# pierrepeterlongo/commet

Hardware: AMD Instinct MI355X
Metric: reads/sec searched (index_and_search, k=32) (higher is better)
Workload: dtype u32

## Files before the change

commet_amd/csrc/capi/search_dispatch.hpp:

```cpp
#pragma once

namespace {

inline int t_eff(const commet_ctx *c, const commet_readset *rs)
{
    return (int) std::min<uint64_t>((uint64_t) c->t, (uint64_t) rs->max_len / (uint64_t) c->k + 1);
}

int launch_search(commet_ctx *c, const commet_readset *rs, const uint64_t *d_sel, uint64_t *d_tags, uint64_t *d_found,
                  unsigned long long *d_counters, unsigned long long *d_probes = nullptr, ActiveList al = ActiveList{nullptr, nullptr},
                  uint64_t n_launch = 0)
{
    if (rs->n_reads == 0) return 0;
    if (al.ids && n_launch == 0) return 0;
    const uint64_t blocks = ((al.ids ? n_launch : rs->n_reads) + 255) / 256;
    if (blocks >= (1ull << 24)) return fail("search launch too large (>= 2^32 reads in one set)");
    const dim3 g((unsigned) blocks), b(256);
    KScope ks(c, "search_kernel", c->stream);
    with_key(c->k, [&](auto key) {
        with_value<false, true>(d_probes != nullptr, [&](auto count) {
            COMMET_LAUNCH((search_kernel<decltype(key), count>), g, b, 0, c->stream, rs->view(), c->view(), c->k, t_eff(c, rs), d_sel, d_tags,
                          d_found, d_counters, d_probes, al);
        });
    });
    HIP_OK(hipGetLastError());
    return 0;
}

int ensure_slots(commet_ctx *c, int g, int gs)
{
    if (c->n_slots < g) {
        HIP_OK(hipStreamSynchronize(c->stream));
        uint32_t *nf = nullptr;
        int want = std::max(g, gs);
        hipError_t e = dev_alloc(c, (void **) &nf, (size_t) want * c->filter_bytes, true);
        if (e != hipSuccess && want > g) {
            (void) hipGetLastError();
            want = g;
            e = dev_alloc(c, (void **) &nf, (size_t) want * c->filter_bytes, true);
        }
        if (e != hipSuccess) return fail("cannot allocate %d filter slots: %s", g, hipGetErrorString(e));
        (void) dm_free(c->filter);
        c->filter = nf;
        c->n_slots = want;
    }
    if (c->il_stride < gs) {
        HIP_OK(hipStreamSynchronize(c->stream));
        (void) dm_free(c->il_a);
        c->il_a = nullptr;
        c->il_stride = 0;
        HIP_OK(dev_alloc(c, (void **) &c->il_a, (size_t) gs * c->plane_words * sizeof(uint32_t), true));
        c->il_stride = gs;
    }
    return 0;
}

int launch_interleave(commet_ctx *c, int g, int gs)
{
    const uint64_t blocks = std::min<uint64_t>((c->plane_words + 255) / 256, 1u << 16);
    KScope ks(c, "interleave_a_kernel", c->stream);
    with_value<2, 4, 8>(gs, [&](auto GS) {
        COMMET_LAUNCH(interleave_a_kernel<GS>, dim3((unsigned) blocks), dim3(256), 0, c->stream, c->filter, 4 * c->plane_words, c->plane_words,
                      g, c->il_a);
    });
    HIP_OK(hipGetLastError());
    return 0;
}

template <typename W, int GS>
int launch_search_group_t(commet_ctx *c, const commet_readset *rs, const FilterGroupView &fg, uint32_t nw_max, const uint64_t *d_sel,
                          uint64_t *d_tags, unsigned long long *d_counters, uint32_t cstride, unsigned long long *d_probes, ActiveList al,
                          uint64_t n_launch)
{
    const dim3 g((unsigned) (((al.ids ? n_launch : rs->n_reads) + 255) / 256)), b(256);
    size_t lds = (size_t) fg.g * 2 * nw_max * 256 * sizeof(uint32_t);
    uint32_t rw_nw = 0;
    if (!d_probes && nw_max <= 8 && lds + (size_t) 3 * nw_max * 256 * sizeof(uint32_t) <= (64u << 10)) {
        rw_nw = nw_max;
        lds += (size_t) 3 * nw_max * 256 * sizeof(uint32_t);
    }
    KScope ks(c, "search_group_kernel", c->stream);
    return with_value<false, true>(d_probes != nullptr, [&](auto count) {
        HIP_OK(hipFuncSetAttribute((const void *) search_group_kernel<W, GS, count>, hipFuncAttributeMaxDynamicSharedMemorySize, (int) lds));
        COMMET_LAUNCH((search_group_kernel<W, GS, count>), g, b, lds, c->stream, rs->view(), fg, c->k, t_eff(c, rs), nw_max, d_sel, d_tags,
                      d_counters, cstride, d_probes, rw_nw, al);
        HIP_OK(hipGetLastError());
        return 0;
    });
}

constexpr int MASK_MAX_WIN = 255;
inline int mask_words(const commet_ctx *c, const commet_readset *rs)
{
    const int64_t fhw = (int64_t) rs->max_len - (int64_t) t_eff(c, rs) * c->k + 1;
    return fhw <= 64 ? 2 : fhw <= 96 ? 3 : fhw <= 128 ? 4 : fhw <= 192 ? 6 : 8;
}
template <typename F>
decltype(auto) with_mask_words(int mw, F &&f)
{
    return with_value<2, 3, 4, 6, 8>(mw, f);
}

int launch_search_group(commet_ctx *c, const commet_readset *rs, int g, int gs, const uint64_t *d_sel, uint64_t *d_tags,
                        unsigned long long *d_counters, uint32_t cstride, unsigned long long *d_probes, ActiveList al = ActiveList{nullptr, nullptr},
                        uint64_t n_launch = 0, uint32_t job_mask = 0, uint64_t job_tag_words = 0)
{
    if (rs->n_reads == 0) return 0;
    if (al.ids && n_launch == 0) return 0;
    if ((rs->n_reads + 255) / 256 >= (1ull << 24)) return fail("search launch too large (>= 2^32 reads in one set)");
    FilterGroupView fg;
    fg.il_a = c->il_a;
    fg.slot0 = c->filter;
    fg.slot_words = 4 * c->plane_words;
    fg.plane_words = c->plane_words;
    fg.g = g;
    if (gs == 8) {
        const int mw_set = mask_words(c, rs);
        auto launch = [&](int mw, ActiveList l, uint64_t n_l) {
            KScope ks(c, "search_group8_kernel", c->stream);
            const dim3 grid((unsigned) (((l.ids ? n_l : rs->n_reads) + 255) / 256)), block(256);
            with_key(c->k, [&](auto key) {
                with_mask_words(mw, [&](auto MW) {
                    COMMET_LAUNCH((search_group8_kernel<decltype(key), MW>), grid, block, 0, c->stream, rs->view(), fg, c->k, t_eff(c, rs), d_sel,
                                  d_tags, d_counters, cstride, l, job_mask, job_tag_words);
                });
            });
        };
        if (al.ids && al.ids == rs->d_len_order && rs->n_len_seg > 1 && !c->mask_split) {
            for (int sg = 0; sg < rs->n_len_seg; ++sg) {
                const commet_readset::LenSeg &seg = rs->len_seg[sg];
                launch(std::min(seg.mw, mw_set), ActiveList{rs->d_len_order + seg.start, rs->d_len_order + rs->n_reads + 1 + sg}, seg.count);
            }
        } else {
            launch(mw_set, al, n_launch);
        }
        HIP_OK(hipGetLastError());
        return 0;
    }
    const uint32_t nw_max = (rs->max_len + 31) / 32;
    return with_key(c->k, [&](auto key) {
        return with_value<2, 4>(gs, [&](auto GS) {
            return launch_search_group_t<decltype(key), GS>(c, rs, fg, nw_max, d_sel, d_tags, d_counters, cstride, d_probes, al, n_launch);
        });
    });
}

bool group_searchable(const commet_ctx *c, const commet_readset *rs, int g)
{
    const uint64_t nw = ((uint64_t) rs->max_len + 31) / 32;
    return c->k >= 2 && nw >= 1 && (uint64_t) g * 2 * nw * 256 * 4 <= (64u << 10);
}

bool group8_ok(const commet_ctx *c, const commet_readset *rs)
{
    const int64_t first_hit_windows = (int64_t) rs->max_len - (int64_t) t_eff(c, rs) * c->k + 1;
    return c->k >= 2 && !c->count_probes && first_hit_windows <= MASK_MAX_WIN;
}

constexpr uint32_t LONG_MIN_MAX_LEN = 5000;
bool long_ok(const commet_ctx *c, const commet_readset *rs)
{
    if (c->long_search == 1 || c->k < 2 || rs->n_reads == 0) return false;
    if (c->long_search == 2) return true;
    const int64_t first_hit_windows = (int64_t) rs->max_len - (int64_t) t_eff(c, rs) * c->k + 1;
    if (first_hit_windows <= MASK_MAX_WIN) return false;
    return rs->max_len >= LONG_MIN_MAX_LEN;
}


int launch_search_long(commet_ctx *c, const commet_readset *rs, int g, int nf, const uint64_t *d_sel, uint64_t *d_tags,
                       unsigned long long *d_counters, uint32_t cstride, unsigned long long *d_probes, ActiveList al, uint64_t n_launch)
{
    if (rs->n_reads == 0) return 0;
    if (al.ids && n_launch == 0) return 0;
    if (g < 1 || g > nf) return fail("internal error: %d filters in a long-read pass of stride %d", g, nf);
    FilterGroupView fg;
    fg.il_a = nf == 1 ? c->slot_ptr(0) : c->il_a;
    fg.slot0 = c->filter;
    fg.slot_words = 4 * c->plane_words;
    fg.plane_words = c->plane_words;
    fg.g = g;
    const uint64_t items = al.ids ? n_launch : rs->n_reads;
    KScope ks(c, "search_long_kernel", c->stream);
    with_key(c->k, [&](auto key) {
        with_value<1, 2, 4, 8>(nf, [&](auto NF) {
            with_value<false, true>(d_probes != nullptr, [&](auto count) {
                static std::atomic<int> resident{0};
                int wgs = resident.load(std::memory_order_relaxed);
                if (!wgs) {
                    int per_cu = 0, cus = 0;
                    if (hipOccupancyMaxActiveBlocksPerMultiprocessor(&per_cu, search_long_kernel<decltype(key), NF, count>, LONG_WG, 0) != hipSuccess ||
                        hipDeviceGetAttribute(&cus, hipDeviceAttributeMultiprocessorCount, c->device) != hipSuccess || per_cu < 1 || cus < 1) {
                        (void) hipGetLastError();
                        per_cu = 4, cus = 256;
                    }
                    wgs = per_cu * cus;
                    resident.store(wgs, std::memory_order_relaxed);
                }
                const uint64_t blocks = std::min<uint64_t>((items + 3) / 4, (uint64_t) wgs);
                COMMET_LAUNCH((search_long_kernel<decltype(key), NF, count>), dim3((unsigned) blocks), dim3(LONG_WG), 0, c->stream, rs->view(), fg,
                              c->k, t_eff(c, rs), d_sel, d_tags, d_counters, cstride, d_probes, al);
            });
        });
    });
    HIP_OK(hipGetLastError());
    return 0;
}

bool sparse_pass(const commet_ctx *c, const commet_readset *rs, const uint64_t *d_sel, uint64_t selected)
{
    if (!d_sel || c->sparse_search == 1 || c->count_probes || rs->n_reads >= (1ull << 32)) return false;
    if (c->sparse_search == 2) return true;
    return rs->n_reads >= 4096 && selected * 2 < rs->n_reads;
}

int build_active_list(commet_ctx *c, const commet_readset *rs, const uint64_t *d_sel, const uint64_t *d_tags, uint64_t selected, ActiveList *al)
{
    const uint64_t n_words = bitmap_words(rs->n_reads), nb = (n_words + IDS_BLOCK_WORDS - 1) / IDS_BLOCK_WORDS;
    if (c->act_cap < selected || c->actblk_cap < nb + 1) {
        if (hipStreamSynchronize(c->stream) != hipSuccess) return 1;
        (void) dm_free(c->d_act), (void) dm_free(c->d_actblk);
        c->d_act = c->d_actblk = nullptr, c->act_cap = c->actblk_cap = 0;
        const uint64_t cap = std::max<uint64_t>(selected, 1024);
        if (dev_alloc(c, (void **) &c->d_act, cap * sizeof(uint32_t), true) != hipSuccess ||
            dev_alloc(c, (void **) &c->d_actblk, (nb + 1) * sizeof(uint32_t), true) != hipSuccess) {
            (void) hipGetLastError();
            (void) dm_free(c->d_act), (void) dm_free(c->d_actblk);
            c->d_act = c->d_actblk = nullptr;
            return 1;
        }
        c->act_cap = cap, c->actblk_cap = nb + 1;
    }
    KScope ks(c, "active_list_kernels", c->stream);
    COMMET_LAUNCH(sel_count_kernel, dim3((unsigned) nb), dim3(64), 0, c->stream, d_sel, n_words, c->d_actblk, d_tags);
    COMMET_LAUNCH(sel_scan_kernel, dim3(1), dim3(1024), 0, c->stream, c->d_actblk, (uint32_t) nb);
    COMMET_LAUNCH(sel_ids_kernel, dim3((unsigned) nb), dim3(64), 0, c->stream, d_sel, n_words, c->d_actblk, c->d_act, d_tags);
    if (hipGetLastError() != hipSuccess) return 1;
    al->ids = c->d_act;
    al->n = c->d_actblk + nb;
    return 0;
}

bool ordered_pass(commet_ctx *c, const commet_readset *rs, const uint64_t *d_sel, bool tags_empty, ActiveList *al)
{
    if (c->ordered_scan == 1 || rs->uniform_len != 0 || d_sel || !tags_empty || al->ids || c->count_probes || rs->len_order_failed) return false;
    if (rs->n_reads == 0 || rs->n_reads >= (1ull << 32) - 1 || (c->ordered_scan == 0 && rs->n_reads < (1u << 16))) return false;
    if (!rs->d_len_order) {
        const uint64_t n_blocks = (rs->n_reads + LO_BLOCK - 1) / LO_BLOCK, entries = n_blocks * LO_CLASSES;
        const uint32_t nb = (uint32_t) ((entries + 4095) / 4096);
        uint32_t *ids = nullptr;
        hipError_t e = dm_malloc((void **) &ids, (rs->n_reads + 8) * sizeof(uint32_t));
        if (e == hipSuccess && c->lo_cnt_cap < entries + 1 + nb + 2) {
            (void) dm_free(c->d_lo_cnt);
            c->d_lo_cnt = nullptr, c->lo_cnt_cap = 0;
            e = dm_malloc((void **) &c->d_lo_cnt, (entries + 1 + nb + 2) * sizeof(unsigned long long));
            if (e == hipSuccess) c->lo_cnt_cap = entries + 1 + nb + 2;
        }
        if (e != hipSuccess) {
            (void) hipGetLastError();
            (void) dm_free(ids);
            rs->len_order_failed = true;
            return false;
        }
        unsigned long long *cnt = c->d_lo_cnt, *totals = cnt + entries + 1;
        const uint32_t tk = (uint32_t) std::min<int64_t>((int64_t) t_eff(c, rs) * c->k, 0x7FFFFFFF);
        KScope ks(c, "len_order_kernels", c->stream);
        COMMET_LAUNCH(lo_count_kernel, dim3((unsigned) n_blocks), dim3(256), 0, c->stream, rs->view(), tk, n_blocks, cnt);
        COMMET_LAUNCH(tq_scan_blocks_kernel, dim3(nb), dim3(1024), 0, c->stream, cnt, entries, totals);
        COMMET_LAUNCH(tq_scan_totals_kernel, dim3(1), dim3(1024), 0, c->stream, totals, nb, totals + nb);
        COMMET_LAUNCH(tq_scan_add_kernel, dim3(nb), dim3(1024), 0, c->stream, cnt, entries, totals, totals + nb);
        COMMET_LAUNCH(lo_fill_kernel, dim3((unsigned) n_blocks), dim3(256), 0, c->stream, rs->view(), tk, n_blocks, cnt, ids);
        if (hipGetLastError() != hipSuccess) {
            (void) hipStreamSynchronize(c->stream);
            (void) dm_free(ids);
            rs->len_order_failed = true;
            return false;
        }
        rs->n_len_seg = 0;
        unsigned long long first[4] = {0, 0, 0, 0};
        static const uint32_t cls[4] = {8, 16, 20, 24};
        static const int width[5] = {8, 6, 4, 3, 2};
        bool ok = true;
        for (int i = 0; i < 4 && ok; ++i)
            ok = hipMemcpyAsync(&first[i], cnt + (uint64_t) cls[i] * n_blocks, sizeof first[i], hipMemcpyDeviceToHost, c->stream) == hipSuccess;
        ok = ok && hipStreamSynchronize(c->stream) == hipSuccess;
        if (ok) {
            const uint64_t bound[6] = {0, first[0], first[1], first[2], first[3], rs->n_reads};
            const uint64_t few = c->ordered_scan == 2 ? 1 : 4096;
            for (int i = 0; i < 5; ++i) {
                const uint64_t a = bound[i], b = bound[i + 1];
                if (b <= a || b > rs->n_reads) continue;
                if (rs->n_len_seg > 0 && b - a < few)
                    rs->len_seg[rs->n_len_seg - 1].count += (uint32_t) (b - a);
                else
                    rs->len_seg[rs->n_len_seg++] = commet_readset::LenSeg{(uint32_t) a, (uint32_t) (b - a), width[i]};
            }
            uint32_t counts[5] = {0, 0, 0, 0, 0};
            for (int i = 0; i < rs->n_len_seg; ++i) counts[i] = rs->len_seg[i].count;
            ok = hipMemcpyAsync(ids + rs->n_reads + 1, counts, sizeof counts, hipMemcpyHostToDevice, c->stream) == hipSuccess &&
                 hipStreamSynchronize(c->stream) == hipSuccess;
        }
        if (!ok) {
            (void) hipGetLastError();
            rs->n_len_seg = 0;
        }
        rs->d_len_order = ids;
    }
    al->ids = rs->d_len_order;
    al->n = rs->d_len_order + rs->n_reads;
    return true;
}

constexpr int TQ_SLICE_BITS = 24;

constexpr int TQ_MAX_K = 34;

bool tiled_ok(const commet_ctx *c, const commet_readset *rs, int g)
{
    if (c->tiled_mode == 1 || c->count_probes || rs->ql.failed) return false;
    if (c->k <= TQ_SLICE_BITS || c->k > TQ_MAX_K || g < 1 || g > 2) return false;
    const int64_t first_hit_windows = (int64_t) rs->max_len - (int64_t) t_eff(c, rs) * c->k + 1;
    if (first_hit_windows < 1 || first_hit_windows > TQ_MAX_WIN) return false;
    if (rs->max_len >= TQ_MAX_LEN) return false;
    if (rs->n_reads >= (1ull << 32)) return false;
    if (rs->fhw_total >= (1ull << 32)) return false;
    if (c->tiled_mode == 2) return true;
    const uint64_t est = rs->fhw_total * 8;
    const bool set_aside = rs->ql_reserved.load() && rs->ql_reserved_at.load() == g_devmem.trims.load();
    if (rs->n_reads < (1ull << 20) || (est > c->ql_max_list && !set_aside)) return false;
    if (est > (4ull << 30) && !rs->ql.built && rs->ql_wanted++ == 0) return false;
    return true;
}

int build_query_list(commet_ctx *c, const commet_readset *rs)
{
    commet_readset::QueryList &ql = rs->ql;
    if (ql.built) {
        ql.last_use = ++c->ql_clock;
        return 0;
    }
    ql.sbits = TQ_SLICE_BITS;
    ql.n_slices = 1u << (c->k - ql.sbits);
    ql.n_pieces = (uint32_t) ((rs->n_reads + TQ_PIECE - 1) / TQ_PIECE);
    const uint64_t entries = (uint64_t) ql.n_slices * ql.n_pieces;
    const uint32_t nb = (uint32_t) ((entries + 4095) / 4096);
    hipStream_t ls = c->list_stream;
    unsigned long long *d_totals = nullptr;
    auto alloc = [&](void **ptr, size_t bytes) -> hipError_t {
        hipError_t ae = dm_malloc(ptr, bytes);
        if (ae != hipErrorOutOfMemory) return ae;
        (void) hipGetLastError();
        if (!shrink_query_lists(c, 0, false)) return ae;
        ae = dm_malloc(ptr, bytes);
        if (ae == hipErrorOutOfMemory) (void) hipGetLastError();
        return ae;
    };
    hipError_t e = alloc((void **) &ql.d_tile_off, (entries + 1) * sizeof(unsigned long long));
    if (e == hipSuccess && c->ql_totals_cap < (uint64_t) nb + 1) {
        (void) dm_free(c->d_ql_totals);
        c->d_ql_totals = nullptr, c->ql_totals_cap = 0;
        e = alloc((void **) &c->d_ql_totals, ((size_t) nb + 1) * sizeof(unsigned long long));
        if (e == hipSuccess) c->ql_totals_cap = (uint64_t) nb + 1;
    }
    d_totals = c->d_ql_totals;
    if (e == hipSuccess) {
        const int t = t_eff(c, rs);
        const size_t lds = (size_t) ql.n_slices * 4;
        {
            KScope ks(c, "tq_count_kernel", ls);
            with_key(c->k, [&](auto key) {
                COMMET_LAUNCH(tq_count_kernel<decltype(key)>, dim3(ql.n_pieces), dim3(256), lds, ls, rs->view(), c->k, t, ql.sbits, ql.n_slices,
                              ql.n_pieces, ql.d_tile_off);
            });
        }
        {
            KScope ks(c, "tq_scan_kernels", ls);
            COMMET_LAUNCH(tq_scan_blocks_kernel, dim3(nb), dim3(1024), 0, ls, ql.d_tile_off, entries, d_totals);
            COMMET_LAUNCH(tq_scan_totals_kernel, dim3(1), dim3(1024), 0, ls, d_totals, nb, d_totals + nb);
            COMMET_LAUNCH(tq_scan_add_kernel, dim3(nb), dim3(1024), 0, ls, ql.d_tile_off, entries, d_totals, d_totals + nb);
        }
        e = hipGetLastError();
        unsigned long long total = 0;
        if (e == hipSuccess) e = hipMemcpyAsync(&total, d_totals + nb, sizeof total, hipMemcpyDeviceToHost, ls);
        if (e == hipSuccess) e = hipStreamSynchronize(ls);
        ql.n_records = total;
        if (e == hipSuccess && total >= (1ull << 32)) e = hipErrorOutOfMemory;
        if (e == hipSuccess) e = alloc((void **) &ql.d_qaddr, std::max<uint64_t>(total, 1) * 4);
        if (e == hipSuccess) e = alloc((void **) &ql.d_qwho, std::max<uint64_t>(total, 1) * 2);
        if (e == hipSuccess) e = alloc((void **) &ql.d_tstart, std::max<uint64_t>(entries, 1) * 4);
        if (e == hipSuccess) e = alloc((void **) &ql.d_tlen, std::max<uint64_t>(entries, 1) * 2);
        if (e == hipSuccess) {
            KScope ks(c, "tq_bounds_kernel", ls);
            COMMET_LAUNCH(tq_bounds_kernel, dim3((unsigned) ((entries + 255) / 256)), dim3(256), 0, ls, ql.d_tile_off, ql.n_slices,
                               ql.n_pieces, ql.d_tstart, ql.d_tlen);
            e = hipGetLastError();
        }
        if (e == hipSuccess) {
            const int64_t fhw = std::max<int64_t>(1, (int64_t) rs->max_len - (int64_t) t * c->k + 1);
            const uint32_t rounds = (uint32_t) (((uint64_t) TQ_PIECE * (uint64_t) fhw + TQ_FILL_CAP - 1) / TQ_FILL_CAP);
            uint32_t rpr = (TQ_PIECE + rounds - 1) / rounds;
            while (rpr > 1 && (uint64_t) rpr * (uint64_t) fhw > TQ_FILL_CAP) --rpr;
            const size_t lds_fill = ((size_t) 4 * ql.n_slices + 2 * TQ_FILL_CAP) * 4;
            e = with_key(c->k, [&](auto key) {
                hipError_t fe = hipFuncSetAttribute((const void *) tq_fill_kernel<decltype(key)>, hipFuncAttributeMaxDynamicSharedMemorySize, (int) lds_fill);
                if (fe != hipSuccess) return fe;
                KScope ks(c, "tq_fill_kernel", ls);
                COMMET_LAUNCH(tq_fill_kernel<decltype(key)>, dim3(ql.n_pieces), dim3(256), lds_fill, ls, rs->view(), c->k, t, ql.sbits, ql.n_slices,
                              ql.n_pieces, rpr, ql.d_tstart, ql.d_qaddr, ql.d_qwho);
                return hipGetLastError();
            });
        }
    }
    if (e == hipSuccess) e = hipEventRecord(c->ev_list, ls);
    if (e == hipSuccess) e = hipStreamWaitEvent(c->stream, c->ev_list, 0);
    if (e != hipSuccess) {
        (void) hipGetLastError();
        ql.release();
        ql.failed = true;
        return 1;
    }
    ql.built = true;
    ql.bytes = (entries + 1) * 8 + ql.n_records * 6 + entries * 6;
    ql.last_use = ++c->ql_clock;
    c->ql_bytes += ql.bytes;
    if (c->ql_bytes > c->ql_budget) (void) shrink_query_lists(c, c->ql_budget, false);
    return 0;
}

int ensure_query_results(commet_ctx *c, const commet_readset *rs)
{
    const uint64_t need = rs->ql.n_records;
    if (c->qres_cap >= need && c->d_qres) return 0;
    if (hipStreamSynchronize(c->stream) != hipSuccess) return 1;
    (void) dm_free(c->d_qres);
    c->d_qres = nullptr, c->qres_cap = 0;
    hipError_t e = dm_malloc((void **) &c->d_qres, std::max<uint64_t>(need, 1));
    if (e == hipErrorOutOfMemory) {
        (void) hipGetLastError();
        if (shrink_query_lists(c, 0, false)) e = dm_malloc((void **) &c->d_qres, std::max<uint64_t>(need, 1));
    }
    if (e != hipSuccess) {
        (void) hipGetLastError();
        rs->ql.failed = true;
        return 1;
    }
    c->qres_cap = need;
    return 0;
}

bool query_list_blocks(const commet_ctx *c, const commet_readset *rs, uint64_t out[6])
{
    const int t = t_eff(c, rs);
    const int64_t fhw = (int64_t) rs->max_len - (int64_t) t * c->k + 1;
    if (c->k <= TQ_SLICE_BITS || c->k > TQ_MAX_K || fhw < 1 || fhw > TQ_MAX_WIN || rs->max_len >= TQ_MAX_LEN || rs->n_reads < (1ull << 20) || rs->n_reads >= (1ull << 32)) return false;
    const uint64_t records = rs->fhw_total;
    if (records >= (1ull << 32)) return false;
    const uint64_t entries = ((uint64_t) 1 << (c->k - TQ_SLICE_BITS)) * ((rs->n_reads + TQ_PIECE - 1) / TQ_PIECE);
    out[0] = (entries + 1) * 8, out[1] = records * 4, out[2] = records * 2, out[3] = entries * 4, out[4] = entries * 2;
    out[5] = c->qres_cap >= records ? 0 : records;
    return true;
}

constexpr unsigned TQ_PROBE_WGS_PER_XCD = 64;

int launch_search_tiled(commet_ctx *c, const commet_readset *rs, int g, int slot0, const uint64_t *d_sel, uint64_t *d_tags,
                        unsigned long long *d_counters, uint32_t cstride, uint64_t job_tag_words = 0)
{
    if (rs->n_reads == 0) return 0;
    const commet_readset::QueryList &q = rs->ql;
    if (c->qres_cap < q.n_records) return fail("internal error: tiled search without its result buffer");
    QueryListView v;
    v.tile_off = q.d_tile_off, v.qaddr = q.d_qaddr, v.qwho = q.d_qwho, v.tstart = q.d_tstart, v.tlen = q.d_tlen;
    v.n_slices = q.n_slices, v.n_pieces = q.n_pieces, v.sbits = q.sbits;
    FilterGroupView fg;
    fg.slot0 = c->slot_ptr(slot0);
    fg.il_a = g == 1 ? c->slot_ptr(slot0) : c->il_a;
    fg.slot_words = 4 * c->plane_words;
    fg.plane_words = c->plane_words;
    fg.g = g;
    const int mw = mask_words(c, rs);
    const int t = t_eff(c, rs);
    {
        KScope ks(c, "tq_probe_kernel", c->stream);
        with_value<1, 2>(g, [&](auto GS) {
            COMMET_LAUNCH(tq_probe_kernel<GS>, dim3(8 * TQ_PROBE_WGS_PER_XCD), dim3(256), 0, c->stream, v, fg.il_a, c->d_qres, 0u, q.n_pieces);
        });
    }
    HIP_OK(hipGetLastError());
    {
        KScope ks(c, "tq_replay_kernel", c->stream);
        const uint32_t hit_cap = (uint32_t) std::min<int>(c->tq_hit_cap, TQ_HIT_CAP);
        with_key(c->k, [&](auto key) {
            with_value<1, 2>(g, [&](auto GS) {
                with_mask_words(mw, [&](auto MW) {
                    COMMET_LAUNCH((tq_replay_kernel<decltype(key), GS, MW>), dim3(q.n_pieces), dim3(TQ_PIECE), 0, c->stream, rs->view(), v, c->d_qres,
                                  fg, c->k, t, d_sel, d_tags, d_counters, cstride, 0u, hit_cap, job_tag_words);
                });
            });
        });
    }
    HIP_OK(hipGetLastError());
    return 0;
}

int slice_words(const commet_ctx *c, uint64_t n_chunks)
{
    if (c->slice_mode == 1 || c->count_probes) return 0;
    if (c->k < SLICE_MIN_K || c->k > SLICE_MAX_K || n_chunks == 0) return 0;
    if (c->slice_mode == 0 && n_chunks < 8) return 0;
    int gw = c->slice_gw ? c->slice_gw : n_chunks > 128 ? 8 : n_chunks > 64 ? 4 : n_chunks > 32 ? 2 : 1;
    while (gw > 1 && (((uint64_t) 16 * gw) << c->k) > (1ull << 30)) gw /= 2;
    return gw;
}

int ensure_slice_buffers(commet_ctx *c, int gw, uint64_t n_chunks)
{
    const uint64_t G = 32ull * gw;
    const uint64_t stage_words = (G * 4) << (c->k - 5), table_words = ((uint64_t) 4 * gw) << c->k;
    if (c->slice_stage_words < stage_words || c->slice_table_words < table_words || c->slice_chunks_cap < n_chunks) {
        HIP_OK(hipStreamSynchronize(c->stream));
        if (c->slice_stage_words < stage_words) {
            (void) dm_free(c->slice_stage);
            c->slice_stage = nullptr, c->slice_stage_words = 0;
            HIP_OK(dev_alloc(c, (void **) &c->slice_stage, stage_words * 4, true));
            c->slice_stage_words = stage_words;
        }
        if (c->slice_table_words < table_words) {
            (void) dm_free(c->slice_tables);
            c->slice_tables = nullptr, c->slice_table_words = 0;
            HIP_OK(dev_alloc(c, (void **) &c->slice_tables, table_words * 4, true));
            c->slice_table_words = table_words;
        }
        if (c->slice_chunks_cap < n_chunks) {
            (void) dm_free(c->d_slice_chunks);
            c->d_slice_chunks = nullptr, c->slice_chunks_cap = 0;
            HIP_OK(dev_alloc(c, (void **) &c->d_slice_chunks, n_chunks * sizeof(SliceChunk), true));
            c->slice_chunks_cap = n_chunks;
        }
    }
    return 0;
}

int launch_slice_build(commet_ctx *c, const commet_readset *rs, const uint64_t *d_sel, uint64_t ci, int g, int gw,
                       uint32_t *tables = nullptr, uint32_t row_words = 0, uint32_t col0 = 0)
{
    if (!tables) tables = c->slice_tables, row_words = (uint32_t) gw, col0 = 0;
    const int tile_bits = std::min(c->k, SLICE_TILE_BITS);
    const uint32_t tiles = 1u << (c->k - tile_bits);
    const size_t lds = (size_t) 4 << (tile_bits - 5);
    HIP_OK(hipFuncSetAttribute((const void *) slice_build_kernel, hipFuncAttributeMaxDynamicSharedMemorySize, (int) lds));
    {
        KScope ks(c, "slice_build_kernel", c->stream);
        COMMET_LAUNCH(slice_build_kernel, dim3(4 * tiles, (unsigned) g), dim3(1024), lds, c->stream, rs->view(), d_sel,
                           c->d_slice_chunks + ci, c->k, tile_bits, tiles, c->slice_stage);
    }
    HIP_OK(hipGetLastError());
    const unsigned grid = (unsigned) ((((uint64_t) 4 << (c->k - 5)) + 255) / 256);
    {
        KScope ks(c, "slice_transpose_kernel", c->stream);
        with_value<1, 2, 4, 8>(gw, [&](auto GW) {
            COMMET_LAUNCH(slice_transpose_kernel<GW>, dim3(grid), dim3(256), 0, c->stream, c->slice_stage, c->k, g, tables, row_words, col0);
        });
    }
    HIP_OK(hipGetLastError());
    return 0;
}

int launch_search_sliced(commet_ctx *c, const commet_readset *rs, int g, int gw, const uint64_t *d_sel, uint64_t *d_tags,
                         unsigned long long *d_counters, uint32_t cstride, uint32_t block_stride = 1)
{
    if (rs->n_reads == 0) return 0;
    if ((rs->n_reads + 255) / 256 >= (1ull << 24)) return fail("search launch too large (>= 2^32 reads in one set)");
    const uint64_t blocks = (rs->n_reads + 255) / 256;
    const dim3 grid((unsigned) ((blocks + block_stride - 1) / block_stride)), block(256);
    KScope ks(c, "search_sliced_kernel", c->stream);
    with_value<1, 2, 4, 8>(gw, [&](auto GW) {
        COMMET_LAUNCH(search_sliced_kernel<GW>, grid, block, 0, c->stream, rs->view(), c->slice_tables, c->k, t_eff(c, rs), g, d_sel, d_tags,
                      d_counters, cstride, block_stride);
    });
    HIP_OK(hipGetLastError());
    return 0;
}

struct WidePlan {
    uint32_t nw = 0;
    uint32_t rw = 0;
    uint64_t chunks_per_pass = 0;
    int lpr = 0, np = 0;
};

WidePlan wide_plan(const commet_ctx *c, uint64_t n_chunks, int slice_gw)
{
    WidePlan w;
    if (!slice_gw || c->slice_wide == 1) return w;
    if (c->slice_wide == 0 && n_chunks <= 256) return w;
    const uint64_t groups = (n_chunks + 255) / 256;
    size_t free_b = 0, total_b = 0;
    if (hipMemGetInfo(&free_b, &total_b) != hipSuccess) return w;
    const uint64_t have = (uint64_t) c->wide_table_words * 4 + dm_filed_bytes(c->device);
    const uint64_t budget = std::min<uint64_t>(((uint64_t) free_b + have) / 3, 48ull << 30);
    uint64_t cap = std::min<uint64_t>(WIDE_MAX_ROW_WORDS, budget / (16ull << c->k));
    if (c->wide_cap_words) cap = std::min<uint64_t>(cap, c->wide_cap_words);
    cap = cap / WIDE_GROUP_WORDS * WIDE_GROUP_WORDS;
    if (cap < WIDE_GROUP_WORDS) return w;
    const uint64_t passes = (groups * WIDE_GROUP_WORDS + cap - 1) / cap;
    const uint64_t groups_per_pass = (groups + passes - 1) / passes;
    w.nw = (uint32_t) (groups_per_pass * WIDE_GROUP_WORDS);
    w.rw = (w.nw + 31u) & ~31u;
    w.chunks_per_pass = groups_per_pass * 256;
    const uint32_t pieces = w.nw / 4;
    w.lpr = pieces <= 8 ? 8 : pieces <= 16 ? 16 : pieces <= 32 ? 32 : 64;
    w.np = pieces <= 64 ? 1 : 2;
    return w;
}

int ensure_wide_tables(commet_ctx *c, const WidePlan &w)
{
    const uint64_t words = ((uint64_t) 4 * w.rw) << c->k;
    if (c->wide_table_words >= words) return 0;
    HIP_OK(hipStreamSynchronize(c->stream));
    (void) dm_free(c->wide_tables);
    c->wide_tables = nullptr, c->wide_table_words = 0;
    if (dev_alloc(c, (void **) &c->wide_tables, words * 4, true) != hipSuccess) {
        (void) hipGetLastError();
        return 1;
    }
    c->wide_table_words = words;
    return 0;
}

int launch_search_wide(commet_ctx *c, const commet_readset *rs, const WidePlan &w, int g, const uint64_t *d_sel, uint64_t *d_tags,
                       unsigned long long *d_counters, uint32_t cstride)
{
    if (rs->n_reads == 0) return 0;
    const uint64_t reads_per_block = 4ull * (64 / w.lpr);
    const uint64_t blocks = (rs->n_reads + reads_per_block - 1) / reads_per_block;
    if (blocks >= (1ull << 31)) return fail("search launch too large");
    const dim3 grid((unsigned) blocks), block(256);
    const int t = t_eff(c, rs);
    KScope ks(c, "search_wide_kernel", c->stream);
    auto launch = [&](auto LPR, auto NP) {
        COMMET_LAUNCH((search_wide_kernel<LPR, NP>), grid, block, 0, c->stream, rs->view(), c->wide_tables, c->k, t, g, w.nw, w.rw, d_sel, d_tags,
                      d_counters, cstride);
    };
    if (w.np == 2) launch(std::integral_constant<int, 64>{}, std::integral_constant<int, 2>{});
    else with_value<64, 32, 16, 8>(w.lpr, [&](auto LPR) { launch(LPR, std::integral_constant<int, 1>{}); });
    HIP_OK(hipGetLastError());
    return 0;
}

}

extern "C" {

uint64_t commet_readset_cache_estimate(commet_ctx *c, const commet_readset *rs)
{
    uint64_t b[6];
    if (rs->ctx != c || !rs->finalized || !query_list_blocks(c, rs, b)) return 0;
    return b[0] + b[1] + b[2] + b[3] + b[4];
}

int commet_readset_reserve_cache(commet_ctx *c, const commet_readset *rs)
{
    if (rs->ctx != c) return fail("read set belongs to another context");
    if (!rs->finalized) return fail("read set not finalized");
    SetUse use(c, rs);
    if (use.enter()) return 1;
    HIP_OK(hipSetDevice(c->device));
    uint64_t b[6];
    {
        std::lock_guard<std::mutex> lk(c->ql_mu);
        const bool still = rs->ql_reserved.load() && rs->ql_reserved_at.load() == g_devmem.trims.load();
        if (rs->ql.built || still || !g_devmem.enabled() || !query_list_blocks(c, rs, b)) return 0;
    }
    for (int i = 0; i < 6; ++i)
        if (b[i] && dm_reserve((size_t) b[i]) != hipSuccess) return 0;
    rs->ql_reserved_at.store(g_devmem.trims.load());
    rs->ql_reserved.store(true);
    return 0;
}

}
```

commet_amd/csrc/capi/state.hpp:

```cpp
#pragma once

using namespace commet;

namespace {

thread_local std::string g_err;

std::mutex g_launch_mu;
std::set<const void *> g_launched;
inline void note_launch(const void *entry)
{
    thread_local const void *recent[16] = {nullptr};
    thread_local unsigned next = 0;
    for (const void *r : recent)
        if (r == entry) return;
    recent[next++ & 15u] = entry;
    std::lock_guard<std::mutex> lk(g_launch_mu);
    g_launched.insert(entry);
}
#define COMMET_LAUNCH(kernel, ...)                                   \
    do {                                                              \
        static std::atomic<bool> noted_{false};                       \
        if (!noted_.load(std::memory_order_relaxed)) {                \
            note_launch((const void *) (kernel));                     \
            noted_.store(true, std::memory_order_relaxed);            \
        }                                                             \
        hipLaunchKernelGGL(kernel, __VA_ARGS__);                      \
    } while (0)

template <typename F>
decltype(auto) with_key(int k, F &&f)
{
    if (k <= 32) return f(uint32_t{});
    return f(uint64_t{});
}
template <auto V, auto... Vs, typename T, typename F>
decltype(auto) with_value(T v, F &&f)
{
    if constexpr (sizeof...(Vs) == 0) {
        return f(std::integral_constant<decltype(V), V>{});
    } else {
        if (v == V) return f(std::integral_constant<decltype(V), V>{});
        return with_value<Vs...>(v, f);
    }
}

struct DevMemCache {
    struct Block {
        int device;
        size_t bytes;
        bool pooled;
    };
    std::mutex mu;
    std::map<void *, Block> live;
    std::multimap<size_t, std::pair<void *, bool>> filed[16];
    size_t filed_bytes[16] = {0};
    size_t cap[16] = {0};
    hipStream_t pool_stream[16] = {nullptr};
    int on = -1, pool_on = -1;
    size_t pool_min = 0;
    std::atomic<uint64_t> drv_ns[16], drv_bytes[16], drv_calls[16];
    std::atomic<uint64_t> trims{0};
    DevMemCache()
    {
        for (int d = 0; d < 16; ++d) drv_ns[d] = 0, drv_bytes[d] = 0, drv_calls[d] = 0;
    }
    bool enabled()
    {
        if (on < 0) {
            const char *e = getenv("COMMET_DEVMEM_CACHE");
            on = !(e && atoi(e) == 0);
        }
        return on != 0;
    }
    int verb = -1;
    bool verbose()
    {
        if (verb < 0) {
            const char *e = getenv("COMMET_DEVMEM_VERBOSE");
            verb = e && atoi(e) != 0;
        }
        return verb != 0;
    }
    bool pooling()
    {
        if (pool_on < 0) {
            const char *e = getenv("COMMET_DEVMEM_POOL");
            pool_on = e && atoi(e) != 0;
            const char *m = getenv("COMMET_DEVMEM_POOL_MIN_MB");
            pool_min = m ? std::max<size_t>((size_t) atoll(m) << 20, (size_t) 8 << 20) : (size_t) 256 << 20;
        }
        return pool_on != 0;
    }
};
DevMemCache g_devmem;
constexpr size_t DEVMEM_MIN_FILED = (size_t) 8 << 20;

hipError_t dm_driver_alloc_untimed(void **p, size_t bytes, int dev, bool shareable, bool *pooled);
hipError_t dm_driver_alloc(void **p, size_t bytes, int dev, bool shareable, bool *pooled)
{
    const auto t0 = std::chrono::steady_clock::now();
    const hipError_t e = dm_driver_alloc_untimed(p, bytes, dev, shareable, pooled);
    if (dev >= 0 && dev < 16) {
        g_devmem.drv_ns[dev] += (uint64_t) std::chrono::duration_cast<std::chrono::nanoseconds>(std::chrono::steady_clock::now() - t0).count();
        g_devmem.drv_calls[dev] += 1;
        if (e == hipSuccess) g_devmem.drv_bytes[dev] += bytes;
    }
    return e;
}
hipError_t dm_driver_alloc_untimed(void **p, size_t bytes, int dev, bool shareable, bool *pooled)
{
    *pooled = false;
    if (!shareable && g_devmem.pooling() && bytes >= g_devmem.pool_min) {
        hipStream_t st;
        {
            std::lock_guard<std::mutex> lk(g_devmem.mu);
            if (!g_devmem.pool_stream[dev] && hipStreamCreateWithFlags(&g_devmem.pool_stream[dev], hipStreamNonBlocking) != hipSuccess) {
                (void) hipGetLastError();
                g_devmem.pool_stream[dev] = nullptr;
            }
            st = g_devmem.pool_stream[dev];
        }
        if (st) {
            hipError_t e = hipMallocAsync(p, bytes, st);
            if (e == hipSuccess) e = hipStreamSynchronize(st);
            if (e == hipSuccess) {
                *pooled = true;
                return e;
            }
            if (e != hipErrorOutOfMemory) (void) hipGetLastError();
            else return e;
        }
    }
    return hipMalloc(p, bytes);
}

void dm_driver_free(void *q, int dev, bool pooled)
{
    if (!pooled) {
        (void) hipFree(q);
        return;
    }
    hipStream_t st = g_devmem.pool_stream[dev];
    (void) hipFreeAsync(q, st);
    (void) hipStreamSynchronize(st);
}

size_t dm_trim(int device)
{
    g_devmem.trims += 1;
    std::vector<std::pair<int, std::pair<void *, bool>>> drop;
    size_t bytes = 0;
    {
        std::lock_guard<std::mutex> lk(g_devmem.mu);
        for (int d = 0; d < 16; ++d) {
            if (device >= 0 && d != device) continue;
            for (auto &b : g_devmem.filed[d]) drop.push_back({d, b.second}), bytes += b.first;
            g_devmem.filed[d].clear();
            g_devmem.filed_bytes[d] = 0;
        }
    }
    bool any_pooled = false;
    for (auto &q : drop) dm_driver_free(q.second.first, q.first, q.second.second), any_pooled |= q.second.second;
    if (any_pooled) {
        int cur = 0;
        const bool have = hipGetDevice(&cur) == hipSuccess;
        for (int d = 0; d < 16; ++d) {
            if ((device >= 0 && d != device) || !g_devmem.pool_stream[d]) continue;
            hipMemPool_t pool;
            if (hipSetDevice(d) == hipSuccess && hipDeviceGetDefaultMemPool(&pool, d) == hipSuccess) (void) hipMemPoolTrimTo(pool, 0);
        }
        if (have) (void) hipSetDevice(cur);
        (void) hipGetLastError();
    }
    return bytes;
}

size_t dm_filed_bytes(int device)
{
    std::lock_guard<std::mutex> lk(g_devmem.mu);
    return device >= 0 && device < 16 ? g_devmem.filed_bytes[device] : 0;
}

size_t dm_pooled_bytes(int device)
{
    std::lock_guard<std::mutex> lk(g_devmem.mu);
    size_t n = 0;
    for (auto &b : g_devmem.live)
        if (b.second.device == device && b.second.pooled) n += b.second.bytes;
    return n;
}

inline size_t dm_size_class(size_t bytes)
{
    if (bytes < DEVMEM_MIN_FILED) return bytes;
    const int lg = 63 - __builtin_clzll((unsigned long long) bytes);
    const size_t granule = (size_t) 1 << (lg - 4);
    return (bytes + granule - 1) & ~(granule - 1);
}

hipError_t dm_malloc(void **p, size_t bytes, bool shareable = false)
{
    *p = nullptr;
    if (g_devmem.enabled()) bytes = dm_size_class(bytes);
    int dev = 0;
    if (hipGetDevice(&dev) != hipSuccess || dev < 0 || dev >= 16) return hipMalloc(p, bytes);
    if (!g_devmem.enabled()) {
        const auto t0 = std::chrono::steady_clock::now();
        const hipError_t e = hipMalloc(p, bytes);
        g_devmem.drv_ns[dev] += (uint64_t) std::chrono::duration_cast<std::chrono::nanoseconds>(std::chrono::steady_clock::now() - t0).count();
        g_devmem.drv_calls[dev] += 1;
        if (e == hipSuccess) g_devmem.drv_bytes[dev] += bytes;
        return e;
    }
    if (bytes >= DEVMEM_MIN_FILED) {
        std::lock_guard<std::mutex> lk(g_devmem.mu);
        for (auto it = g_devmem.filed[dev].lower_bound(bytes); it != g_devmem.filed[dev].end() && it->first <= bytes + bytes / 4; ++it) {
            if (shareable && it->second.second) continue;
            *p = it->second.first;
            g_devmem.filed_bytes[dev] -= it->first;
            g_devmem.live[*p] = {dev, it->first, it->second.second};
            g_devmem.filed[dev].erase(it);
            return hipSuccess;
        }
    }
    bool pooled = false;
    if (g_devmem.verbose()) {
        std::lock_guard<std::mutex> lk(g_devmem.mu);
        fprintf(stderr, "[devmem] driver alloc %.1f MiB (filed: %.1f GiB in %zu blocks)\n", bytes / 1048576.0, g_devmem.filed_bytes[dev] / 1073741824.0, g_devmem.filed[dev].size());
    }
    hipError_t e = dm_driver_alloc(p, bytes, dev, shareable, &pooled);
    if (e == hipErrorOutOfMemory && dm_trim(dev)) {
        (void) hipGetLastError();
        e = dm_driver_alloc(p, bytes, dev, shareable, &pooled);
    }
    if (e == hipSuccess && bytes >= DEVMEM_MIN_FILED) {
        std::lock_guard<std::mutex> lk(g_devmem.mu);
        g_devmem.live[*p] = {dev, bytes, pooled};
    }
    return e;
}

hipError_t dm_reserve(size_t bytes)
{
    if (!g_devmem.enabled() || bytes < DEVMEM_MIN_FILED) return hipSuccess;
    bytes = dm_size_class(bytes);
    int dev = 0;
    if (hipGetDevice(&dev) != hipSuccess || dev < 0 || dev >= 16) return hipErrorInvalidDevice;
    void *p = nullptr;
    bool pooled = false;
    const hipError_t e = dm_driver_alloc(&p, bytes, dev, false, &pooled);
    if (e != hipSuccess) {
        (void) hipGetLastError();
        return e;
    }
    std::lock_guard<std::mutex> lk(g_devmem.mu);
    g_devmem.filed[dev].emplace(bytes, std::make_pair(p, pooled));
    g_devmem.filed_bytes[dev] += bytes;
    return hipSuccess;
}

hipError_t dm_free(void *p)
{
    if (!p) return hipSuccess;
    if (g_devmem.enabled()) {
        DevMemCache::Block what{-1, 0, false};
        {
            std::lock_guard<std::mutex> lk(g_devmem.mu);
            auto it = g_devmem.live.find(p);
            if (it != g_devmem.live.end()) what = it->second, g_devmem.live.erase(it);
        }
        if (what.device >= 0) {
            const int d = what.device;
            int cur = d;
            const bool have_cur = hipGetDevice(&cur) == hipSuccess;
            if (have_cur && cur != d) (void) hipSetDevice(d);
            (void) hipDeviceSynchronize();
            std::vector<std::pair<void *, bool>> over;
            {
                std::lock_guard<std::mutex> lk(g_devmem.mu);
                g_devmem.filed[d].emplace(what.bytes, std::make_pair(p, what.pooled));
                g_devmem.filed_bytes[d] += what.bytes;
                if (!g_devmem.cap[d]) {
                    size_t fr = 0, tot = 0;
                    const char *e = getenv("COMMET_DEVMEM_CACHE_GB");
                    if (e) g_devmem.cap[d] = (size_t) (std::max(0.0, atof(e)) * (double) (1ull << 30)) + 1;
                    else g_devmem.cap[d] = hipMemGetInfo(&fr, &tot) == hipSuccess ? tot / 2 : (size_t) 64 << 30;
                }
                while (g_devmem.filed_bytes[d] > g_devmem.cap[d] && !g_devmem.filed[d].empty()) {
                    auto last = std::prev(g_devmem.filed[d].end());
                    over.push_back(last->second);
                    g_devmem.filed_bytes[d] -= last->first;
                    g_devmem.filed[d].erase(last);
                }
            }
            if (!over.empty() && g_devmem.verbose()) fprintf(stderr, "[devmem] over the cap of %.1f GiB: %zu block(s) back to the driver\n", g_devmem.cap[d] / 1073741824.0, over.size());
            for (auto &q : over) dm_driver_free(q.first, d, q.second);
            if (have_cur && cur != d) (void) hipSetDevice(cur);
            return hipSuccess;
        }
    }
    return hipFree(p);
}

hipError_t dm_make_shareable(void **p)
{
    if (!*p) return hipSuccess;
    DevMemCache::Block what{-1, 0, false};
    {
        std::lock_guard<std::mutex> lk(g_devmem.mu);
        auto it = g_devmem.live.find(*p);
        if (it != g_devmem.live.end()) what = it->second;
    }
    if (what.device < 0 || !what.pooled) return hipSuccess;
    void *q = nullptr;
    hipError_t e = dm_malloc(&q, what.bytes, true);
    if (e != hipSuccess) return e;
    e = hipDeviceSynchronize();
    if (e == hipSuccess) e = hipMemcpy(q, *p, what.bytes, hipMemcpyDeviceToDevice);
    if (e == hipSuccess) e = hipDeviceSynchronize();
    if (e != hipSuccess) {
        (void) dm_free(q);
        return e;
    }
    (void) dm_free(*p);
    *p = q;
    return hipSuccess;
}

int fail(const char *fmt, ...)
{
    char buf[1024];
    va_list ap;
    va_start(ap, fmt);
    vsnprintf(buf, sizeof buf, fmt, ap);
    va_end(ap);
    g_err = buf;
    return 1;
}

#define HIP_OK(expr)                                                                                   \
    do {                                                                                               \
        hipError_t e_ = (expr);                                                                        \
        if (e_ != hipSuccess) return fail("%s failed: %s (%s:%d)", #expr, hipGetErrorString(e_), __FILE__, __LINE__); \
    } while (0)

#define HIP_OK_NULL(expr)                                                                              \
    do {                                                                                               \
        hipError_t e_ = (expr);                                                                        \
        if (e_ != hipSuccess) {                                                                        \
            fail("%s failed: %s (%s:%d)", #expr, hipGetErrorString(e_), __FILE__, __LINE__);           \
            return nullptr;                                                                            \
        }                                                                                              \
    } while (0)

inline uint64_t bitmap_words(uint64_t n) { return n / 64 + 1; }
inline uint64_t bitmap_bytes_host(uint64_t n) { return n / 8 + 1; }

constexpr uint64_t STAGE_BASES = 64ull << 20;
constexpr uint64_t STAGE_READS = 1ull << 20;
constexpr int      N_COUNTERS = 8;

}

struct commet_ctx {
    int device = 0;
    int k = 0, t = 0;
    hipStream_t stream = nullptr;
    uint32_t *filter = nullptr;
    uint64_t plane_words = 0;
    uint64_t filter_bytes = 0;
    unsigned long long *d_counters = nullptr;
    unsigned long long *h_counters = nullptr;
    hipEvent_t ev_i0 = nullptr, ev_i1 = nullptr, ev_s0 = nullptr, ev_s1 = nullptr;
    bool have_index_ev = false, have_search_ev = false;
    bool count_probes = false;
    int index_mode = 0;
    int part_packed = 1;
    int part_no_uni = 0;
    int part_list = 0;
    uint64_t part_min_kmers = 8ull << 20;
    struct PartWs {
        uint32_t *bufA = nullptr, *bufB = nullptr;
        uint64_t cap_keys = 0, cap_b = 0;
        uint32_t *hist = nullptr, *wl = nullptr;
        uint64_t *off = nullptr, *goff = nullptr;
        unsigned long long *cur2 = nullptr, *blockoff = nullptr;
        uint32_t *blockcnt = nullptr;
        uint32_t *items = nullptr, *itemblk = nullptr;
        uint64_t items_cap = 0, itemblk_cap = 0;
        uint64_t items_set = 0, items_first = 0, items_count = 0;
        uint32_t items_nblk = 0;
        uint32_t nb = 0;
        void release()
        {
            (void) dm_free(bufA); (void) dm_free(bufB); (void) dm_free(hist); (void) dm_free(wl); (void) dm_free(off); (void) dm_free(goff);
            (void) dm_free(cur2); (void) dm_free(blockoff); (void) dm_free(blockcnt); (void) dm_free(items); (void) dm_free(itemblk);
            *this = PartWs();
        }
    } part[2];
    unsigned long long *d_jobcnt = nullptr;
    uint32_t *d_ids = nullptr, *d_idblk = nullptr;
    uint64_t ids_cap = 0, idblk_cap = 0;
    uint32_t *d_ids2 = nullptr, *d_idblk2 = nullptr;
    uint64_t ids2_cap = 0, idblk2_cap = 0;
    uint32_t *d_act = nullptr, *d_actblk = nullptr;
    uint64_t act_cap = 0, actblk_cap = 0;
    uint64_t *d_mtags = nullptr;
    uint64_t mtags_cap = 0;
    int multi_job = 0;
    int sparse_search = 0;
    unsigned long long *d_plansum = nullptr;
    uint64_t plansum_cap = 0;
    uint64_t jobcnt_cap = 0;
    hipStream_t aux_stream = nullptr;
    hipStream_t load_stream = nullptr;
    hipEvent_t ev_fork = nullptr, ev_join = nullptr;
    int index_lanes = 2;
    bool stagger_armed = false;
    hipEvent_t ev_stagger = nullptr;

    int n_slots = 1;
    int cur_slot = 0;
    uint32_t *il_a = nullptr;
    int il_stride = 0;
    struct KernelClock {
        struct Rec { const char *name; hipEvent_t a, b; };
        bool on = false;
        std::vector<Rec> open;
        std::vector<hipEvent_t> spare;
        std::vector<std::string> names;
        std::vector<uint64_t> launches;
        std::vector<double> total_ms;
        std::mutex mu;
        void add(const char *name, double ms)
        {
            std::lock_guard<std::mutex> lk(mu);
            size_t i = 0;
            while (i < names.size() && names[i] != name) ++i;
            if (i == names.size()) names.push_back(name), launches.push_back(0), total_ms.push_back(0);
            launches[i] += 1;
            total_ms[i] += ms;
        }
        hipEvent_t get()
        {
            hipEvent_t e = nullptr;
            if (!spare.empty()) e = spare.back(), spare.pop_back();
            else if (hipEventCreate(&e) != hipSuccess) e = nullptr;
            return e;
        }
        void collect()
        {
            for (Rec &r : open) {
                float ms = 0;
                if (r.a && r.b && hipEventElapsedTime(&ms, r.a, r.b) == hipSuccess) add(r.name, ms);
                if (r.a) spare.push_back(r.a);
                if (r.b) spare.push_back(r.b);
            }
            open.clear();
        }
        void reset()
        {
            std::lock_guard<std::mutex> lk(mu);
            names.clear(), launches.clear(), total_ms.clear();
        }
        void release()
        {
            collect();
            for (hipEvent_t e : spare) (void) hipEventDestroy(e);
            spare.clear();
        }
    } kclock;
    uint32_t *slice_stage = nullptr, *slice_tables = nullptr;
    SliceChunk *d_slice_chunks = nullptr;
    uint64_t slice_stage_words = 0, slice_table_words = 0, slice_chunks_cap = 0;
    hipStream_t list_stream = nullptr;
    hipEvent_t ev_list = nullptr;
    unsigned long long *d_ql_totals = nullptr;
    uint64_t ql_totals_cap = 0;
    uint8_t *d_qres = nullptr;
    uint64_t qres_cap = 0;
    int tq_hit_cap = TQ_HIT_CAP;
    int ordered_scan = 0;
    int mask_split = 0;
    unsigned long long *d_lo_cnt = nullptr;
    uint64_t lo_cnt_cap = 0;
    int tiled_mode = 0;
    bool job_verbose = false;
    bool ingest_verbose = false;
    int slice_mode = 0;
    int slice_gw = 0;
    int slice_wide = 0;
    uint32_t wide_cap_words = 0;
    uint32_t *wide_tables = nullptr;
    uint64_t wide_table_words = 0;
    uint64_t max_kmer_test = 0;
    double *d_shannon = nullptr;
    uint32_t shannon_lo = 0, shannon_hi = 0;
    int long_search = 0;
    int chunk_group = 8;
    struct IngestBuf {
        uint32_t *h_planes = nullptr;
        uint64_t *h_goff = nullptr;
        hipEvent_t done = nullptr;
    };
    std::vector<IngestBuf> ingest_pool;
    struct AwayStage {
        uint8_t *h = nullptr;
        hipEvent_t done = nullptr;
        bool inflight = false;
    } away[2];

    std::mutex ql_mu;
    std::vector<commet_readset *> sets;
    uint64_t ql_bytes = 0, ql_budget = 64ull << 30, ql_clock = 0, ql_evictions = 0;
    uint64_t ql_max_list = 4ull << 30;

    uint32_t *slot_ptr(int i) const { return filter + (uint64_t) i * 4 * plane_words; }
    FilterView view() const
    {
        uint32_t *base = slot_ptr(cur_slot);
        FilterView f;
        f.a = base;
        f.b = base + plane_words;
        f.c = base + 2 * plane_words;
        f.d = base + 3 * plane_words;
        return f;
    }
};

struct commet_readset {
    commet_ctx *ctx = nullptr;
    uint64_t max_reads = 0, max_bases = 0;
    uint64_t n_reads = 0, n_bases = 0;
    uint32_t *d_planes = nullptr;
    uint64_t *d_goff = nullptr;
    uint32_t *d_kcnt = nullptr;
    uint32_t *d_lenmm = nullptr;
    uint64_t *d_sel = nullptr, *d_tags = nullptr, *d_found = nullptr;
    struct Stage {
        uint8_t *h_bases = nullptr;
        uint64_t *h_offs = nullptr;
        uint8_t *d_bases = nullptr;
        uint64_t *d_offs = nullptr;
        hipEvent_t done = nullptr;
        bool inflight = false;
    } st[2];
    int cur = 0;
    bool acquired = false;
    uint64_t stage_bases = 0, stage_reads = 0;
    std::vector<FileSpan> files;
    std::vector<uint64_t> empty_reads;
    mutable std::vector<uint32_t> h_kcnt;
    mutable std::vector<uint64_t> h_kprefix;
    mutable bool have_host_counts = false;
    uint32_t uniform_len = 0;
    uint32_t max_kcnt = 0;
    uint32_t max_len = 0, min_len = 0;
    uint64_t uid = 0;
    uint64_t fhw_total = 0;
    struct QueryList {
        unsigned long long *d_tile_off = nullptr;
        uint32_t *d_qaddr = nullptr, *d_tstart = nullptr;
        uint16_t *d_qwho = nullptr, *d_tlen = nullptr;
        uint64_t n_records = 0;
        uint32_t n_slices = 0, n_pieces = 0;
        int sbits = 0;
        bool built = false, failed = false;
        uint64_t bytes = 0, last_use = 0;
        void release()
        {
            (void) dm_free(d_tile_off); (void) dm_free(d_qaddr); (void) dm_free(d_qwho); (void) dm_free(d_tstart); (void) dm_free(d_tlen);
            *this = QueryList();
        }
    };
    mutable QueryList ql;
    mutable uint32_t *d_len_order = nullptr;
    mutable bool len_order_failed = false;
    struct LenSeg { uint32_t start, count; int mw; };
    mutable LenSeg len_seg[5];
    mutable int n_len_seg = 0;
    mutable uint32_t ql_wanted = 0;
    mutable std::atomic<uint64_t> ql_reserved_at{0};
    mutable std::atomic<bool> ql_reserved{false};
    mutable int in_job = 0;
    mutable uint64_t *d_filter_ws = nullptr;
    mutable uint64_t filter_ws_bytes = 0;
    bool host_packed = false;
    uint32_t host_min_len = 0xFFFFFFFFu, host_max_len = 0;
    bool finalized = false;
    bool resident = true;
    bool moving = false;
    uint8_t *h_away = nullptr;
    uint64_t away_bytes = 0;

    ReadsView view() const
    {
        ReadsView v;
        v.planes = d_planes;
        v.goff = d_goff;
        v.uniform_len = uniform_len;
        v.n = n_reads;
        return v;
    }
};

namespace {
struct SetUse {
    commet_ctx *c;
    std::vector<const commet_readset *> sets;
    bool held = false;
    explicit SetUse(commet_ctx *c_) : c(c_) {}
    SetUse(commet_ctx *c_, const commet_readset *rs) : c(c_), sets(1, rs) {}
    void add(const commet_readset *rs) { sets.push_back(rs); }
    int enter()
    {
        std::lock_guard<std::mutex> lk(c->ql_mu);
        for (const commet_readset *rs : sets)
            if (!rs->resident) return fail("read set is offloaded");
        for (const commet_readset *rs : sets) ++rs->in_job;
        held = true;
        return 0;
    }
    ~SetUse()
    {
        if (!held) return;
        std::lock_guard<std::mutex> lk(c->ql_mu);
        for (const commet_readset *rs : sets) --rs->in_job;
    }
    SetUse(const SetUse &) = delete;
    SetUse &operator=(const SetUse &) = delete;
};

struct KScope {
    commet_ctx::KernelClock &kc;
    hipStream_t stream;
    size_t idx = ~(size_t) 0;
    KScope(commet_ctx *c, const char *name, hipStream_t s) : kc(c->kclock), stream(s)
    {
        if (!kc.on) return;
        commet_ctx::KernelClock::Rec r{name, kc.get(), kc.get()};
        if (r.a) (void) hipEventRecord(r.a, stream);
        idx = kc.open.size();
        kc.open.push_back(r);
    }
    ~KScope()
    {
        if (idx != ~(size_t) 0 && kc.open[idx].b) (void) hipEventRecord(kc.open[idx].b, stream);
    }
};
}
```

commet_amd/csrc/tile_search.hpp:

```cpp
#pragma once

#include "kernels.hpp"
#include "index_part.hpp"

namespace commet {

constexpr int TQ_SWEEP_U = 2;
constexpr int TQ_COLLECT_U = 8;
constexpr int TQ_HIT_CAP = 1024;
constexpr uint32_t TQ_PIECE = 256;
constexpr uint32_t TQ_MAX_LEN = 8000;
constexpr int      TQ_MAX_WIN = 255;

struct QueryListView {
    const unsigned long long *tile_off;
    const uint32_t *qaddr;
    const uint16_t *qwho;
    const uint32_t *tstart;
    const uint16_t *tlen;
    uint32_t n_slices, n_pieces;
    int sbits;
};

template <typename W, typename F>
__device__ __forceinline__ void tq_for_each_window(const ReadsView &rv, uint64_t r, int k, int t, F &&f)
{
    using T = KeyTraits<W>;
    uint64_t t0;
    uint32_t len;
    read_extent(rv, r, t0, len);
    const uint32_t *p = rv.planes + 3 * t0;
    const int pe = (int) len - 1 - (t - 1) * k;
    const int sh = T::BITS - k;
    W wh = 0;
    uint32_t run = 0;
    for (uint32_t w = 0; (int) (w * 32u) <= pe; ++w) {
        const uint32_t hi = p[3 * w], va = p[3 * w + 2];
        const uint32_t nb = (uint32_t) min(32, pe - (int) (w * 32u) + 1);
        for (uint32_t j = 0; j < nb; ++j) {
            wh = (wh >> 1) | ((W) ((hi >> j) & 1u) << (k - 1));
            run = ((va >> j) & 1u) ? run + 1 : 0;
            if (run < (uint32_t) k) continue;
            bool selfp;
            const W addr = psi_a<W>(T::brev(wh) >> sh, k, selfp);
            f(32u * w + j - (uint32_t) (k - 1), addr, selfp);
        }
    }
}

template <typename W>
__global__ __launch_bounds__(256) void tq_count_kernel(ReadsView rv, int k, int t, int sbits, uint32_t n_slices, uint32_t n_pieces,
                                                       unsigned long long *__restrict__ cnt)
{
    extern __shared__ uint32_t h[];
    for (uint32_t i = threadIdx.x; i < n_slices; i += 256) h[i] = 0;
    __syncthreads();
    const uint64_t r0 = (uint64_t) blockIdx.x * TQ_PIECE;
    for (uint32_t i = threadIdx.x; i < TQ_PIECE; i += 256) {
        const uint64_t r = r0 + i;
        if (r >= rv.n) break;
        tq_for_each_window<W>(rv, r, k, t, [&](uint32_t, W addr, bool) { atomicAdd(&h[(uint32_t) (addr >> sbits)], 1u); });
    }
    __syncthreads();
    for (uint32_t s = threadIdx.x; s < n_slices; s += 256) cnt[(uint64_t) s * n_pieces + blockIdx.x] = h[s];
}

__global__ __launch_bounds__(1024) void tq_scan_blocks_kernel(unsigned long long *__restrict__ a, uint64_t n, unsigned long long *__restrict__ totals)
{
    __shared__ unsigned long long wsum[16];
    const uint64_t base = (uint64_t) blockIdx.x * 4096 + threadIdx.x * 4ull;
    unsigned long long v[4], s = 0;
#pragma unroll
    for (int i = 0; i < 4; ++i) {
        v[i] = base + i < n ? a[base + i] : 0ull;
        s += v[i];
    }
    const int lane = threadIdx.x & 63, wave = threadIdx.x >> 6;
    unsigned long long inc = s;
    for (int o = 1; o < 64; o <<= 1) {
        const unsigned long long x = __shfl_up(inc, o, 64);
        if (lane >= o) inc += x;
    }
    if (lane == 63) wsum[wave] = inc;
    __syncthreads();
    unsigned long long wbase = 0, tot = 0;
    for (int i = 0; i < 16; ++i) {
        if (i < wave) wbase += wsum[i];
        tot += wsum[i];
    }
    unsigned long long ex = wbase + inc - s;
#pragma unroll
    for (int i = 0; i < 4; ++i) {
        if (base + i < n) a[base + i] = ex;
        ex += v[i];
    }
    if (threadIdx.x == 0) totals[blockIdx.x] = tot;
}

__global__ __launch_bounds__(1024) void tq_scan_totals_kernel(unsigned long long *__restrict__ totals, uint32_t n_blocks,
                                                              unsigned long long *__restrict__ grand_total)
{
    __shared__ unsigned long long wsum[16];
    __shared__ unsigned long long carry;
    if (threadIdx.x == 0) carry = 0;
    __syncthreads();
    for (uint32_t b0 = 0; b0 < n_blocks; b0 += 1024) {
        const uint32_t i = b0 + threadIdx.x;
        const unsigned long long v = i < n_blocks ? totals[i] : 0ull;
        const int lane = threadIdx.x & 63, wave = threadIdx.x >> 6;
        unsigned long long inc = v;
        for (int o = 1; o < 64; o <<= 1) {
            const unsigned long long x = __shfl_up(inc, o, 64);
            if (lane >= o) inc += x;
        }
        if (lane == 63) wsum[wave] = inc;
        __syncthreads();
        unsigned long long wbase = 0, tot = 0;
        for (int w = 0; w < 16; ++w) {
            if (w < wave) wbase += wsum[w];
            tot += wsum[w];
        }
        const unsigned long long c = carry;
        if (i < n_blocks) totals[i] = c + wbase + inc - v;
        __syncthreads();
        if (threadIdx.x == 0) carry = c + tot;
        __syncthreads();
    }
    if (threadIdx.x == 0) *grand_total = carry;
}

__global__ __launch_bounds__(1024) void tq_scan_add_kernel(unsigned long long *__restrict__ a, uint64_t n, const unsigned long long *__restrict__ totals,
                                                           const unsigned long long *__restrict__ grand_total)
{
    const uint64_t base = (uint64_t) blockIdx.x * 4096 + threadIdx.x * 4ull;
    const unsigned long long add = totals[blockIdx.x];
#pragma unroll
    for (int i = 0; i < 4; ++i)
        if (base + i < n) a[base + i] += add;
    if (blockIdx.x == 0 && threadIdx.x == 0) a[n] = *grand_total;
}

constexpr uint32_t LO_BLOCK = 1024, LO_CLASSES = 32;
__device__ __forceinline__ uint32_t lo_class(const ReadsView &rv, uint64_t r, uint32_t tk)
{
    const uint64_t len = rv.goff[r + 1] - rv.goff[r];
    const uint64_t wins = len >= tk ? len - tk + 1 : 0;
    return LO_CLASSES - 1u - (uint32_t) min(wins / 8, (uint64_t) (LO_CLASSES - 1));
}

__global__ __launch_bounds__(256) void lo_count_kernel(ReadsView rv, uint32_t tk, uint64_t n_blocks, unsigned long long *__restrict__ cnt)
{
    __shared__ uint32_t h[LO_CLASSES];
    if (threadIdx.x < LO_CLASSES) h[threadIdx.x] = 0;
    __syncthreads();
    const uint64_t r0 = (uint64_t) blockIdx.x * LO_BLOCK;
    for (uint32_t i = threadIdx.x; i < LO_BLOCK; i += 256)
        if (r0 + i < rv.n) atomicAdd(&h[lo_class(rv, r0 + i, tk)], 1u);
    __syncthreads();
    if (threadIdx.x < LO_CLASSES) cnt[(uint64_t) threadIdx.x * n_blocks + blockIdx.x] = h[threadIdx.x];
}

__global__ __launch_bounds__(256) void lo_fill_kernel(ReadsView rv, uint32_t tk, uint64_t n_blocks, const unsigned long long *__restrict__ off,
                                                      uint32_t *__restrict__ ids)
{
    __shared__ uint32_t h[LO_CLASSES];
    __shared__ unsigned long long base[LO_CLASSES];
    if (threadIdx.x < LO_CLASSES) {
        h[threadIdx.x] = 0;
        base[threadIdx.x] = off[(uint64_t) threadIdx.x * n_blocks + blockIdx.x];
    }
    __syncthreads();
    const uint64_t r0 = (uint64_t) blockIdx.x * LO_BLOCK;
    for (uint32_t i = threadIdx.x; i < LO_BLOCK; i += 256) {
        const uint64_t r = r0 + i;
        if (r >= rv.n) break;
        const uint32_t c = lo_class(rv, r, tk);
        ids[base[c] + atomicAdd(&h[c], 1u)] = (uint32_t) r;
    }
    if (blockIdx.x == 0 && threadIdx.x == 0) ids[rv.n] = (uint32_t) rv.n;
}

__global__ __launch_bounds__(256) void tq_bounds_kernel(const unsigned long long *__restrict__ tile_off, uint32_t n_slices, uint32_t n_pieces,
                                                        uint32_t *__restrict__ tstart, uint16_t *__restrict__ tlen)
{
    const uint64_t i = blockIdx.x * 256ull + threadIdx.x;
    if (i >= (uint64_t) n_slices * n_pieces) return;
    const uint64_t p = i / n_slices, s = i % n_slices;
    const unsigned long long a = tile_off[s * n_pieces + p], e = tile_off[s * n_pieces + p + 1];
    tstart[i] = (uint32_t) a;
    tlen[i] = (uint16_t) (e - a);
}

constexpr uint32_t TQ_FILL_CAP = 9600;
template <typename W>
__global__ __launch_bounds__(256) void tq_fill_kernel(ReadsView rv, int k, int t, int sbits, uint32_t n_slices, uint32_t n_pieces,
                                                      uint32_t rpr, const uint32_t *__restrict__ tstart,
                                                      uint32_t *__restrict__ qaddr, uint16_t *__restrict__ qwho)
{
    static_assert(TQ_PIECE <= 256 && TQ_MAX_WIN <= 256, "qwho packs the read in 8 bits and the window in 8");
    extern __shared__ uint32_t fl[];
    uint32_t *cnt = fl, *base = cnt + n_slices, *fill = base + n_slices, *dstb = fill + n_slices;
    uint32_t *rec_a = dstb + n_slices, *rec_w = rec_a + TQ_FILL_CAP;
    __shared__ uint32_t wsum[16];
    __shared__ uint32_t pw[TQ_PIECE + 1];
    for (uint32_t i = threadIdx.x; i < n_slices; i += 256) dstb[i] = tstart[(uint64_t) blockIdx.x * n_slices + i];
    const uint64_t r0 = (uint64_t) blockIdx.x * TQ_PIECE;
    const uint32_t smask = (1u << sbits) - 1u;
    {
        uint32_t w = 0;
        if (threadIdx.x < TQ_PIECE && r0 + threadIdx.x < rv.n) {
            uint64_t t0;
            uint32_t len;
            read_extent(rv, r0 + threadIdx.x, t0, len);
            const uint32_t tk = (uint32_t) t * (uint32_t) k;
            w = len >= tk ? len - tk + 1 : 0;
        }
        uint32_t tot;
        const uint32_t ex = block_scan<256>(w, wsum, &tot);
        if (threadIdx.x < TQ_PIECE) pw[threadIdx.x] = ex;
        if (threadIdx.x == 0) pw[TQ_PIECE] = tot;
        __syncthreads();
    }
    (void) rpr;
    for (uint32_t rr = 0, hi = 0; rr < TQ_PIECE; rr = hi) {
        {
            uint32_t lo = rr + 1, up = TQ_PIECE;
            const uint32_t lim = pw[rr] + TQ_FILL_CAP;
            while (lo < up) {
                const uint32_t mid = (lo + up + 1) >> 1;
                if (pw[mid] <= lim) lo = mid;
                else up = mid - 1;
            }
            hi = lo;
        }
        for (uint32_t i = threadIdx.x; i < n_slices; i += 256) cnt[i] = 0, fill[i] = 0;
        __syncthreads();
        const uint32_t i = rr + threadIdx.x;
        const bool mine = i < hi && r0 + i < rv.n;
        if (mine) tq_for_each_window<W>(rv, r0 + i, k, t, [&](uint32_t, W addr, bool) { atomicAdd(&cnt[(uint32_t) (addr >> sbits)], 1u); });
        __syncthreads();
        lds_scan<256>(cnt, base, n_slices, wsum);
        if (mine)
            tq_for_each_window<W>(rv, r0 + i, k, t, [&](uint32_t win, W addr, bool selfp) {
                const uint32_t s = (uint32_t) (addr >> sbits);
                const uint32_t at = base[s] + atomicAdd(&fill[s], 1u);
                rec_a[at] = ((uint32_t) addr & smask) | (selfp ? 0x80000000u : 0u);
                rec_w[at] = i | (win << 8) | (s << 16);
            });
        __syncthreads();
        const uint32_t total = base[n_slices - 1] + cnt[n_slices - 1];
        for (uint32_t j = threadIdx.x; j < total; j += 256) {
            const uint32_t w = rec_w[j], s = w >> 16;
            const uint32_t dst = dstb[s] + (j - base[s]);
            qaddr[dst] = rec_a[j];
            qwho[dst] = (uint16_t) (w & 0xFFFFu);
        }
        __syncthreads();
        for (uint32_t s = threadIdx.x; s < n_slices; s += 256) dstb[s] += cnt[s];
    }
}

template <int GS>
__device__ __forceinline__ uint32_t tq_probe_one(const uint32_t *__restrict__ base, uint32_t q)
{
    const uint32_t addr = q & 0x7FFFFFFFu, bit = addr & 31u;
    const bool selfp = q >> 31;
    if constexpr (GS == 1) {
        const uint32_t wd = base[addr >> 5];
        const uint32_t fb = (wd >> bit) & 1u;
        return fb | ((selfp ? fb : (wd >> (bit ^ 1u)) & 1u) << 1);
    } else {
        const uint2 wd = *(const uint2 *) (base + (uint64_t) (addr >> 5) * 2);
        const uint32_t f0 = (wd.x >> bit) & 1u, f1 = (wd.y >> bit) & 1u;
        const uint32_t r0 = selfp ? f0 : (wd.x >> (bit ^ 1u)) & 1u, r1 = selfp ? f1 : (wd.y >> (bit ^ 1u)) & 1u;
        return f0 | (f1 << 1) | (r0 << 2) | (r1 << 3);
    }
}

template <int GS>
__global__ __launch_bounds__(256) void tq_probe_kernel(QueryListView ql, const uint32_t *__restrict__ planes_a, uint8_t *__restrict__ qres,
                                                       uint32_t p0, uint32_t p1)
{
    const uint32_t x = blockIdx.x % 8, j = blockIdx.x / 8, wpx = gridDim.x / 8;
    const uint32_t s_lo = (uint32_t) ((uint64_t) x * ql.n_slices / 8), s_hi = (uint32_t) ((uint64_t) (x + 1) * ql.n_slices / 8);
    for (uint32_t s = s_lo; s < s_hi; ++s) {
        unsigned long long a = ql.tile_off[(uint64_t) s * ql.n_pieces + p0];
        const unsigned long long e = ql.tile_off[(uint64_t) s * ql.n_pieces + p1];
        const uint32_t *base = planes_a + (((uint64_t) s << ql.sbits) >> 5) * GS;
        const unsigned long long a4 = (a + 3) & ~3ull, e4 = e & ~3ull;
        if (a4 < e4) {
            const unsigned long long step = (unsigned long long) wpx * 256, m_end = e4 / 4;
            unsigned long long m = a4 / 4 + (unsigned long long) j * 256 + threadIdx.x;
            for (; m < m_end; m += step) {
                const uint32_t *qp = ql.qaddr + 4 * m;
                const uint32_t q0 = __builtin_nontemporal_load(qp), q1 = __builtin_nontemporal_load(qp + 1),
                               q2 = __builtin_nontemporal_load(qp + 2), q3 = __builtin_nontemporal_load(qp + 3);
                const uint32_t r = tq_probe_one<GS>(base, q0) | (tq_probe_one<GS>(base, q1) << 8) | (tq_probe_one<GS>(base, q2) << 16) |
                                   (tq_probe_one<GS>(base, q3) << 24);
                __builtin_nontemporal_store(r, (uint32_t *) (qres + 4 * m));
            }
        }
        if (j == 0 && threadIdx.x < 8) {
            unsigned long long i;
            bool mine;
            if (a4 < e4) {
                i = threadIdx.x < 4 ? a + threadIdx.x : e4 + (threadIdx.x - 4);
                mine = threadIdx.x < 4 ? i < a4 : i < e;
            } else {
                i = a + threadIdx.x;
                mine = i < e;
            }
            if (mine) qres[i] = (uint8_t) tq_probe_one<GS>(base, ql.qaddr[i]);
        }
    }
}

template <typename W, int GS, int MW>
__global__ __launch_bounds__(TQ_PIECE) COMMET_SGPRS void tq_replay_kernel(ReadsView rv, QueryListView ql, const uint8_t *__restrict__ qres,
                                                             FilterGroupView fg, int k, int t, const uint64_t *__restrict__ sel,
                                                             uint64_t *__restrict__ tags, unsigned long long *__restrict__ counters,
                                                             uint32_t cstride, uint32_t piece0, uint32_t hit_cap, uint64_t job_tag_words)
{
    const bool multi = GS == 2 && job_tag_words != 0;
    const uint32_t piece = blockIdx.x + piece0;
    __shared__ uint32_t masks[GS * 2 * MW * TQ_PIECE];
    auto mask_at = [&](int c, int strand, int h, uint32_t rd) -> uint32_t & { return masks[(((c * 2 + strand) * MW) + h) * TQ_PIECE + rd]; };
    for (uint32_t i = threadIdx.x; i < GS * 2 * MW * TQ_PIECE; i += TQ_PIECE) masks[i] = 0;
    __syncthreads();
    {
        const uint32_t lane = threadIdx.x & 63, wave = threadIdx.x >> 6;
        constexpr uint32_t NWAVE = TQ_PIECE / 64;
        for (uint32_t s0 = wave; s0 < ql.n_slices; s0 += 64 * NWAVE) {
            const uint32_t sl = s0 + lane * NWAVE;
            unsigned long long ta = 0, te = 0;
            if (sl < ql.n_slices) {
                ta = ql.tstart[(uint64_t) piece * ql.n_slices + sl];
                te = ta + ql.tlen[(uint64_t) piece * ql.n_slices + sl];
            }
            const uint32_t len = (uint32_t) (te - ta);
            uint32_t inc = len;
            for (int o = 1; o < 64; o <<= 1) {
                const uint32_t x = __shfl_up(inc, o, 64);
                if ((int) lane >= o) inc += x;
            }
            const uint32_t total = __shfl(inc, 63, 64);
            for (uint32_t f0 = 0; f0 < total; f0 += 64 * TQ_COLLECT_U) {
                unsigned long long ri[TQ_COLLECT_U];
                bool ok[TQ_COLLECT_U];
#pragma unroll
                for (int u = 0; u < TQ_COLLECT_U; ++u) {
                    const uint32_t f = f0 + 64u * (uint32_t) u + lane;
                    uint32_t lo = 0, hi = 64;
#pragma unroll
                    for (int step = 0; step < 7; ++step) {
                        const uint32_t mid = min((lo + hi) >> 1, 63u);
                        const uint32_t pm = __shfl(inc, (int) mid, 64);
                        if (lo < hi) {
                            if (pm <= f) lo = mid + 1;
                            else hi = mid;
                        }
                    }
                    const uint32_t src = min(lo, 63u);
                    const uint32_t before_raw = __shfl(inc, (int) (src ? src - 1 : 0), 64);
                    const unsigned long long tbase = __shfl((unsigned long long) ta, (int) src, 64);
                    ok[u] = f < total;
                    ri[u] = ok[u] ? tbase + (f - (src ? before_raw : 0u)) : 0ull;
                }
                uint32_t res[TQ_COLLECT_U], who[TQ_COLLECT_U];
#pragma unroll
                for (int u = 0; u < TQ_COLLECT_U; ++u) {
                    res[u] = __builtin_nontemporal_load(qres + ri[u]);
                    who[u] = __builtin_nontemporal_load(ql.qwho + ri[u]);
                }
#pragma unroll
                for (int u = 0; u < TQ_COLLECT_U; ++u) {
                    if (!ok[u] || !res[u]) continue;
                    const uint32_t rd = who[u] & 255u, win = who[u] >> 8;
#pragma unroll
                    for (int c = 0; c < GS; ++c) {
                        if ((res[u] >> c) & 1u) atomicOr(&mask_at(c, 0, (int) (win >> 5), rd), 1u << (win & 31u));
                        if ((res[u] >> (GS + c)) & 1u) atomicOr(&mask_at(c, 1, (int) (win >> 5), rd), 1u << (win & 31u));
                    }
                }
            }
        }
    }
    __syncthreads();
    __shared__ uint32_t hits[TQ_HIT_CAP];
    __shared__ uint32_t hit_n;
    __shared__ uint32_t rd_ext[TQ_PIECE];
    __shared__ unsigned long long piece_t0;
    __shared__ uint32_t pre[TQ_PIECE];
    __shared__ uint32_t scan_ws[TQ_PIECE / 64];
    __shared__ unsigned int wg_cnt[2 * GS];
    constexpr int NS = 2 * GS;
    auto word_at = [&](uint32_t *arr, int i, int h, uint32_t rd) -> uint32_t & { return arr[((i * MW) + h) * TQ_PIECE + rd]; };
    if (threadIdx.x < 2 * GS) wg_cnt[threadIdx.x] = 0;
    if (threadIdx.x == 0) hit_n = 0;
    static_assert(TQ_PIECE == 256, "search_lane, add_chunk_counters and cooperative_tail are written for workgroups of 256 threads");
    const ActiveList no_list{nullptr, nullptr};
    const SearchLane me = search_lane(rv, no_list, sel, multi ? nullptr : tags, piece0);
    const uint64_t r = me.r;
    const bool active = me.active;
    uint64_t my_t0 = 0;
    uint32_t my_len = 0;
    if (r < rv.n) read_extent(rv, r, my_t0, my_len);
    if (threadIdx.x == 0) piece_t0 = my_t0;
    const KeyCtx<W> kc(k);
#pragma unroll
    for (int i = 0; i < NS; ++i)
#pragma unroll
        for (int h = 0; h < MW; ++h)
            if (!active || (i >> 1) >= fg.g) word_at(masks, i, h, threadIdx.x) = 0;
    __syncthreads();
    rd_ext[threadIdx.x] = (r < rv.n) ? ((uint32_t) (my_t0 - piece_t0) & 0xFFFFu) | (my_len << 16) : 0u;
    constexpr uint32_t TQ_HEAVY = 20;
    uint32_t am[NS][MW];
    uint32_t hv = 0;
#pragma unroll
    for (int i = 0; i < NS; ++i) {
        uint32_t n = 0;
#pragma unroll
        for (int h = 0; h < MW; ++h) am[i][h] = word_at(masks, i, h, threadIdx.x), n += __popc(am[i][h]);
        if (n > TQ_HEAVY) {
            hv |= 1u << i;
#pragma unroll
            for (int h = 0; h < MW; ++h) word_at(masks, i, h, threadIdx.x) = 0;
        }
    }
    const uint32_t *const piece_planes = rv.planes + 3 * piece_t0;
    auto keys_of = [&](uint32_t owner, int strand, int q, W &ka, W &kb) {
        (void) kc.window_keys(piece_planes + 3u * (rd_ext[owner] & 0xFFFFu), q, strand, ka, kb);
    };
    auto sweep = [&](uint32_t *src, auto &&word_of, auto &&on_set) {
        uint32_t cnt = 0;
#pragma unroll
        for (int i = 0; i < NS; ++i)
#pragma unroll
            for (int h = 0; h < MW; ++h) cnt += __popc(word_at(src, i, h, threadIdx.x));
        uint32_t total;
        const uint32_t ex = block_scan<TQ_PIECE>(cnt, scan_ws, &total);
        pre[threadIdx.x] = ex + cnt;
        __syncthreads();
        constexpr int U = TQ_SWEEP_U;
        for (uint32_t f0 = threadIdx.x; f0 < total; f0 += U * TQ_PIECE) {
            uint32_t owner[U], bitn[U], fw[U], fbit[U];
            W ka[U], kb[U];
            int sc[U], hw[U];
            bool have[U];
#pragma unroll
            for (int u = 0; u < U; ++u) {
                const uint32_t f = f0 + (uint32_t) u * TQ_PIECE;
                have[u] = f < total;
                owner[u] = 0, bitn[u] = 0, sc[u] = 0, hw[u] = 0;
                if (!have[u]) continue;
                uint32_t lo = 0, hi = TQ_PIECE - 1;
                while (lo < hi) {
                    const uint32_t mid = (lo + hi) >> 1;
                    if (pre[mid] <= f) lo = mid + 1;
                    else hi = mid;
                }
                uint32_t local = f - (lo ? pre[lo - 1] : 0u), wd = 0;
                bool got = false;
#pragma unroll
                for (int i = 0; i < NS; ++i)
#pragma unroll
                    for (int h = 0; h < MW; ++h) {
                        if (got) continue;
                        const uint32_t x = word_at(src, i, h, lo);
                        const uint32_t c = __popc(x);
                        if (local < c) sc[u] = i, hw[u] = h, wd = x, got = true;
                        else local -= c;
                    }
                for (uint32_t v = 0; v < local; ++v) wd &= wd - 1u;
                owner[u] = lo, bitn[u] = (uint32_t) __ffs((int) wd) - 1u;
            }
            const uint32_t *wp[U];
#pragma unroll
            for (int u = 0; u < U; ++u) {
                ka[u] = kb[u] = 0;
                if (have[u]) keys_of(owner[u], sc[u] & 1, (int) (32 * hw[u] + bitn[u]) + (k - 1), ka[u], kb[u]);
            }
#pragma unroll
            for (int u = 0; u < U; ++u) {
                fw[u] = 0, fbit[u] = 0;
                if (have[u]) {
                    wp[u] = word_of(sc[u], ka[u], kb[u], fbit[u]);
                    fw[u] = *wp[u];
                }
            }
#pragma unroll
            for (int u = 0; u < U; ++u)
                if (have[u] && ((fw[u] >> fbit[u]) & 1u)) on_set(owner[u], sc[u], hw[u], bitn[u], ka[u], kb[u]);
        }
        __syncthreads();
    };
    sweep(masks,
          [&](int i, W, W kb, uint32_t &bit) -> const uint32_t * {
              bit = (uint32_t) kb & 31u;
              return fg.slot0 + (uint64_t) (i >> 1) * fg.slot_words + fg.plane_words + (kb >> 5);
          },
          [&](uint32_t owner, int i, int h, uint32_t b, W ka, W kb) {
              const uint32_t *pc = fg.slot0 + (uint64_t) (i >> 1) * fg.slot_words + 2 * fg.plane_words, *pd = pc + fg.plane_words;
              const uint32_t vc = pc[(ka ^ kb) >> 5], vd = pd[(ka | kb) >> 5];
              if ((vc >> ((uint32_t) (ka ^ kb) & 31u)) & (vd >> ((uint32_t) (ka | kb) & 31u)) & 1u) {
                  const uint32_t at = atomicAdd(&hit_n, 1u);
                  if (at < hit_cap) hits[at] = owner | ((uint32_t) i << 8) | ((uint32_t) h << 12) | (b << 16);
              }
          });
#pragma unroll
    for (int i = 0; i < NS; ++i)
#pragma unroll
        for (int h = 0; h < MW; ++h) word_at(masks, i, h, threadIdx.x) = 0;
    __syncthreads();
    const uint32_t nh = hit_n;
    const bool all_self = nh > hit_cap;
    for (uint32_t e = threadIdx.x; e < min(nh, hit_cap); e += TQ_PIECE) {
        const uint32_t x = hits[e];
        atomicOr(&word_at(masks, (int) ((x >> 8) & 15u), (int) ((x >> 12) & 15u), x & 255u), 1u << (x >> 16));
    }
    __syncthreads();
    static_assert(TQ_HIT_CAP >= 2 * TQ_PIECE, "the tails' arrays alias the hit list");
    uint32_t *const tail_req = hits, *const tail_bits = tail_req + TQ_PIECE;
    __shared__ uint32_t tail_n;
    int found_chunk = -1;
    bool found_job0 = false, found_job1 = false;
    {
        const uint32_t *p = rv.planes + 3 * my_t0;
        const int last = (int) my_len - 1;
        const int pe = last - (t - 1) * k;
        const int q0 = k - 1;
        bool found = false;
        for (int i = 0; i < 2 * fg.g; ++i) {
            if (multi && i == 2) found_job0 = found, found = false;
            const int strand = i & 1;
            const PlanesBCD f = planes_bcd(fg, i >> 1);
            StrandScan sc(active && !found);
            auto probe_own = [&](int q) -> bool {
                W ka, kb;
                (void) kc.window_keys(p, q, strand, ka, kb);
                return probe_bcd_together<W>(f, ka, kb);
            };
            const bool hscan = ((hv >> i) & 1u) || all_self;
            for (int h = 0; h < MW && sc.open(); ++h) {
                uint32_t m = masks[((i * MW) + h) * TQ_PIECE + threadIdx.x];
                if (hscan) {
                    m = 0;
#pragma unroll
                    for (int ii = 0; ii < NS; ++ii)
#pragma unroll
                        for (int hh = 0; hh < MW; ++hh)
                            if (ii == i && hh == h) m = am[ii][hh];
                }
                sc.walk(m, q0 + 32 * h, t, k, last, [&](int q) -> bool { return !hscan || probe_own(q); });
            }
            cooperative_tail<W, 32, GS>(
                sc, tail_req, tail_bits, tail_n, kc, strand, t, pe, last, fg.il_a, i >> 1,
                [&](uint32_t owner, int q, W &wh, W &wl) -> bool {
                    const uint32_t oext = rd_ext[owner];
                    if (q >= (int) (oext >> 16)) return false;
                    ItemWords<W> ot;
                    ot.load(piece_planes + 3u * (oext & 0xFFFFu), (uint32_t) q >> 5);
                    return ot.window((uint32_t) q & 31u, k, kc.mask, wh, wl);
                },
                probe_own);
            found = found || sc.found;
            if (found && found_chunk < 0) found_chunk = i >> 1;
        }
        found_job1 = found;
    }
    const int lane = threadIdx.x & 63;
    const uint64_t word = me.word;
    const bool in_range = me.in_range;
    if constexpr (GS == 2) if (multi) {
        const uint64_t fb0 = __ballot(found_job0), fb1 = __ballot(found_job1), sc = __ballot(active);
        if (lane == 0 && in_range && tags) tags[word] = fb0, tags[job_tag_words + word] = fb1;
        __syncthreads();
        if (counters) {
            if (lane == 0) {
                if (sc) atomicAdd(&wg_cnt[0], (unsigned int) __popcll(sc)), atomicAdd(&wg_cnt[2], (unsigned int) __popcll(sc));
                if (fb0) atomicAdd(&wg_cnt[1], (unsigned int) __popcll(fb0));
                if (fb1) atomicAdd(&wg_cnt[3], (unsigned int) __popcll(fb1));
            }
            __syncthreads();
            if (threadIdx.x < 4u && wg_cnt[threadIdx.x])
                atomicAdd(&counters[(uint64_t) (threadIdx.x >> 1) * cstride + (threadIdx.x & 1)], (unsigned long long) wg_cnt[threadIdx.x]);
        }
        return;
    }
    publish_found(no_list, me, found_chunk >= 0, tags);
    if (counters) add_chunk_counters(counters, cstride, fg.g, active, found_chunk, wg_cnt);
}

}
```

commet_amd/lib.py:

```python
import ctypes as C
import os

_HERE = os.path.dirname(os.path.abspath(__file__))
LIB_PATH = os.path.join(_HERE, "libcommet_hip.so")

u8p = C.POINTER(C.c_uint8)
u32p = C.POINTER(C.c_uint32)
u64p = C.POINTER(C.c_uint64)
f64p = C.POINTER(C.c_double)


class PairStats(C.Structure):
    _fields_ = [("indexed", C.c_uint64), ("searched", C.c_uint64), ("shared", C.c_uint64),
                ("search_ms", C.c_double)]


class JobInfo(C.Structure):
    _fields_ = [("n_chunks", C.c_uint64), ("kmers_indexed", C.c_uint64), ("reads_scanned", C.c_uint64),
                ("reads_indexed", C.c_uint64), ("index_launches", C.c_uint64), ("search_launches", C.c_uint64),
                ("probes", C.c_uint64), ("zero_ms", C.c_double), ("index_ms", C.c_double),
                ("index_kernel_ms", C.c_double), ("search_ms", C.c_double), ("total_ms", C.c_double)]


class FilterStats(C.Structure):
    _fields_ = [("reads", C.c_uint64), ("selected", C.c_uint64), ("removed_length", C.c_uint64), ("removed_n", C.c_uint64),
                ("removed_shannon", C.c_uint64)]


class KernelTime(C.Structure):
    _fields_ = [("name", C.c_char * 48), ("launches", C.c_uint64), ("total_ms", C.c_double)]


SIGNATURES = {
    "commet_version": (C.c_char_p, []),
    "commet_last_error": (C.c_char_p, []),
    "commet_device_count": (C.c_int, []),
    "commet_create": (C.c_void_p, [C.c_int, C.c_int, C.c_int]),
    "commet_destroy": (None, [C.c_void_p]),
    "commet_kmer_size": (C.c_int, [C.c_void_p]),
    "commet_min_hits": (C.c_int, [C.c_void_p]),
    "commet_max_kmer": (C.c_uint64, [C.c_void_p]),
    "commet_synchronize": (C.c_int, [C.c_void_p]),
    "commet_device_memory": (C.c_int, [C.c_void_p, u64p, u64p]),
    "commet_readset_create": (C.c_void_p, [C.c_void_p, C.c_uint64, C.c_uint64]),
    "commet_readset_destroy": (None, [C.c_void_p]),
    "commet_readset_begin_file": (C.c_int, [C.c_void_p]),
    "commet_readset_stage_acquire": (C.c_int, [C.c_void_p, C.POINTER(u8p), u64p, C.POINTER(u64p), u64p]),
    "commet_readset_stage_commit": (C.c_int, [C.c_void_p, C.c_uint64]),
    "commet_readset_append": (C.c_int, [C.c_void_p, C.c_void_p, C.c_void_p, C.c_uint64]),
    "commet_readset_from_fasta": (C.c_void_p, [C.c_void_p, C.POINTER(C.c_char_p), C.c_int]),
    "commet_readset_from_buffers": (C.c_void_p, [C.c_void_p, C.POINTER(C.c_char_p), u64p, C.c_int]),
    "commet_readset_save": (C.c_int, [C.c_void_p, C.c_char_p]),
    "commet_readset_load": (C.c_void_p, [C.c_void_p, C.c_char_p]),
    "commet_readset_export": (C.c_int, [C.c_void_p, C.c_void_p, C.c_uint64, u64p]),
    "commet_readset_import": (C.c_void_p, [C.c_void_p, C.c_void_p, C.c_uint64]),
    "commet_readset_file_reads": (C.c_uint64, [C.c_void_p, C.c_uint64]),
    "commet_readset_finalize": (C.c_int, [C.c_void_p]),
    "commet_readset_num_reads": (C.c_uint64, [C.c_void_p]),
    "commet_readset_num_files": (C.c_uint64, [C.c_void_p]),
    "commet_readset_kmer_counts": (C.c_int, [C.c_void_p, C.c_void_p]),
    "commet_readset_filter": (C.c_int, [C.c_void_p, C.c_void_p, C.c_int, C.c_int64, C.c_float, C.c_int64, C.c_void_p,
                                        C.POINTER(FilterStats)]),
    "commet_readset_offload": (C.c_int, [C.c_void_p]),
    "commet_readset_restore": (C.c_int, [C.c_void_p]),
    "commet_readset_is_resident": (C.c_int, [C.c_void_p]),
    "commet_readset_device_bytes": (C.c_uint64, [C.c_void_p]),
    "commet_readset_packed_bytes": (C.c_uint64, [C.c_void_p]),
    "commet_files_packed_bytes": (C.c_int, [C.POINTER(C.c_char_p), C.c_int, u64p, u64p, u64p]),
    "commet_readset_cache_bytes": (C.c_uint64, [C.c_void_p]),
    "commet_readset_drop_cache": (None, [C.c_void_p]),
    "commet_cache_stats": (C.c_int, [C.c_void_p, u64p, u64p, u64p]),
    "commet_readset_cache_estimate": (C.c_uint64, [C.c_void_p, C.c_void_p]),
    "commet_readset_reserve_cache": (C.c_int, [C.c_void_p, C.c_void_p]),
    "commet_device_cache_trim": (C.c_uint64, [C.c_int]),
    "commet_device_cache_bytes": (C.c_uint64, [C.c_int]),
    "commet_device_pooled_bytes": (C.c_uint64, [C.c_int]),
    "commet_device_alloc_stats": (C.c_int, [C.c_int, C.POINTER(C.c_double), u64p, u64p]),
    "commet_filter_reset": (C.c_int, [C.c_void_p]),
    "commet_index_reads": (C.c_int, [C.c_void_p, C.c_void_p, C.c_uint64, C.c_uint64, C.c_void_p, u64p]),
    "commet_search_reads": (C.c_int, [C.c_void_p, C.c_void_p, C.c_void_p, C.c_void_p, u64p, u64p]),
    "commet_index_and_search": (C.c_int, [C.c_void_p, C.c_void_p, C.c_void_p, C.c_int, C.POINTER(C.c_void_p),
                                          C.POINTER(C.c_void_p), C.POINTER(C.c_void_p), C.POINTER(PairStats),
                                          C.POINTER(JobInfo)]),
    "commet_index_many_and_search": (C.c_int, [C.c_void_p, C.c_int, C.POINTER(C.c_void_p), C.POINTER(C.c_void_p), C.c_void_p, C.c_void_p,
                                               C.POINTER(C.c_void_p), C.POINTER(PairStats), C.POINTER(JobInfo)]),
    "commet_set_option": (C.c_int, [C.c_void_p, C.c_char_p, C.c_int64]),
    "commet_filter_export_reference": (C.c_int, [C.c_void_p, C.c_void_p, C.c_uint64]),
    "commet_last_kernel_ms": (C.c_int, [C.c_void_p, f64p, f64p]),
    "commet_kernel_times": (C.c_int, [C.c_void_p, C.POINTER(KernelTime), C.c_int, C.POINTER(C.c_int)]),
    "commet_launched_kernels": (C.c_int, [C.POINTER(C.c_void_p), C.c_int, C.POINTER(C.c_int)]),
    "commet_membench": (C.c_int, [C.c_void_p, C.c_int, C.c_uint64, C.c_uint64, f64p]),
    "commet_ldsbench": (C.c_int, [C.c_void_p, C.c_int, C.c_uint32, C.c_uint64, f64p]),
}

_lib = None


def load():
    global _lib
    if _lib is not None:
        return _lib
    if not os.path.exists(LIB_PATH):
        raise RuntimeError(
            f"{LIB_PATH} is missing: build it with `python -m commet_amd.build` "
            "(hipcc --offload-arch=gfx950). There is no CPU fallback for this path.")
    lib = C.CDLL(LIB_PATH, mode=C.RTLD_LOCAL)
    for name, (res, args) in SIGNATURES.items():
        fn = getattr(lib, name)
        fn.restype = res
        fn.argtypes = args
    _lib = lib
    return lib
```

include/commet_hip.h:

```cpp
#ifndef COMMET_HIP_H_
#define COMMET_HIP_H_

#include <stddef.h>
#include <stdint.h>

#ifdef __cplusplus
extern "C" {
#endif

typedef struct commet_ctx     commet_ctx;
typedef struct commet_readset commet_readset;

const char *commet_version(void);
const char *commet_last_error(void);
int         commet_device_count(void);

commet_ctx *commet_create(int device, int kmer_size, int min_hits);
void        commet_destroy(commet_ctx *ctx);
int         commet_kmer_size(const commet_ctx *ctx);
int         commet_min_hits(const commet_ctx *ctx);
uint64_t    commet_max_kmer(const commet_ctx *ctx);
int         commet_device_memory(const commet_ctx *ctx, uint64_t *free_bytes, uint64_t *total_bytes);
int         commet_synchronize(commet_ctx *ctx);

commet_readset *commet_readset_create(commet_ctx *ctx, uint64_t max_reads, uint64_t max_bases);
void            commet_readset_destroy(commet_readset *rs);
int             commet_readset_begin_file(commet_readset *rs);
int             commet_readset_stage_acquire(commet_readset *rs, uint8_t **bases, uint64_t *bases_cap,
                                             uint64_t **offsets, uint64_t *reads_cap);
int             commet_readset_stage_commit(commet_readset *rs, uint64_t n_reads);
int             commet_readset_append(commet_readset *rs, const uint8_t *bases, const uint64_t *offsets,
                                      uint64_t n_reads);
commet_readset *commet_readset_from_fasta(commet_ctx *ctx, const char *const *paths, int n_paths);
commet_readset *commet_readset_from_buffers(commet_ctx *ctx, const char *const *data, const uint64_t *sizes, int n_files);
uint64_t        commet_readset_file_reads(const commet_readset *rs, uint64_t file_index);
int             commet_readset_finalize(commet_readset *rs);
int             commet_readset_save(const commet_readset *rs, const char *path);
commet_readset *commet_readset_load(commet_ctx *ctx, const char *path);
int             commet_readset_export(const commet_readset *rs, void *blob, uint64_t cap, uint64_t *blob_bytes);
commet_readset *commet_readset_import(commet_ctx *ctx, const void *blob, uint64_t blob_bytes);
uint64_t        commet_readset_num_reads(const commet_readset *rs);
uint64_t        commet_readset_num_files(const commet_readset *rs);
int             commet_readset_kmer_counts(const commet_readset *rs, uint32_t *kmers_out);
typedef struct {
    uint64_t reads;
    uint64_t selected;
    uint64_t removed_length;
    uint64_t removed_n;
    uint64_t removed_shannon;
} commet_filter_stats;
int             commet_readset_filter(commet_ctx *ctx, const commet_readset *rs, int min_len, int64_t max_n ,
                                      float min_shannon, int64_t max_reads_per_file ,
                                      uint8_t *select_out , commet_filter_stats *per_file );
uint64_t        commet_readset_cache_bytes(const commet_readset *rs);
void            commet_readset_drop_cache(commet_readset *rs);
int             commet_cache_stats(commet_ctx *ctx, uint64_t *bytes, uint64_t *budget_bytes, uint64_t *evictions);
int             commet_readset_offload(commet_readset *rs);
int             commet_readset_restore(commet_readset *rs);
int             commet_readset_is_resident(const commet_readset *rs);
uint64_t        commet_readset_device_bytes(const commet_readset *rs);
uint64_t        commet_readset_packed_bytes(const commet_readset *rs);
int             commet_files_packed_bytes(const char *const *paths, int n_paths, uint64_t *reads, uint64_t *bases, uint64_t *packed_bytes);
uint64_t        commet_device_cache_trim(int device);
uint64_t        commet_readset_cache_estimate(commet_ctx *ctx, const commet_readset *rs);
int             commet_readset_reserve_cache(commet_ctx *ctx, const commet_readset *rs);
uint64_t        commet_device_cache_bytes(int device);
uint64_t        commet_device_pooled_bytes(int device);
int             commet_device_alloc_stats(int device, double *wait_ms, uint64_t *fresh_bytes, uint64_t *calls);

int commet_filter_reset(commet_ctx *ctx);

int commet_index_reads(commet_ctx *ctx, const commet_readset *rs, uint64_t first, uint64_t count,
                       const uint8_t *select_bits, uint64_t *kmers_fed);

int commet_search_reads(commet_ctx *ctx, const commet_readset *rs, const uint8_t *active_bits,
                        uint8_t *found_bits, uint64_t *n_scanned, uint64_t *n_found);

typedef struct {
    uint64_t indexed;
    uint64_t searched;
    uint64_t shared;
    double   search_ms;
} commet_pair_stats;

typedef struct {
    uint64_t n_chunks;
    uint64_t kmers_indexed;
    uint64_t reads_scanned;
    uint64_t reads_indexed;
    uint64_t index_launches;
    uint64_t search_launches;
    uint64_t probes;
    double   zero_ms;
    double   index_ms;
    double   index_kernel_ms;
    double   search_ms;
    double   total_ms;
} commet_job_info;

int commet_index_and_search(commet_ctx *ctx,
                            const commet_readset *index_rs, const uint8_t *index_select,
                            int n_search, const commet_readset *const *search_rs,
                            const uint8_t *const *search_select,
                            uint8_t *const *tags_out, commet_pair_stats *stats,
                            commet_job_info *info);
int commet_index_many_and_search(commet_ctx *ctx, int n_jobs, const commet_readset *const *index_rs,
                                 const uint8_t *const *index_select, const commet_readset *search_rs,
                                 const uint8_t *search_select, uint8_t *const *tags_out, commet_pair_stats *stats,
                                 commet_job_info *info);

int commet_set_option(commet_ctx *ctx, const char *name, int64_t value);
int commet_filter_export_reference(commet_ctx *ctx, uint8_t *out, uint64_t out_bytes);
int commet_last_kernel_ms(commet_ctx *ctx, double *index_ms, double *search_ms);
typedef struct {
    char     name[48];
    uint64_t launches;
    double   total_ms;
} commet_kernel_time;
int commet_kernel_times(commet_ctx *ctx, commet_kernel_time *out, int cap, int *n_out);
int commet_launched_kernels(const void **out, int cap, int *n_out);
int commet_membench(commet_ctx *ctx, int atomic, uint64_t table_bytes, uint64_t n_access, double *ms);
int commet_ldsbench(commet_ctx *ctx, int mode, uint32_t n_words, uint64_t n_access, double *ms);

#ifdef __cplusplus
}
#endif
#endif
```

Before: 527.1 million.

## Repack tiled query list into padded per-piece layout with tile deltas

Restructures the tiled query list so that each piece's results and read/window ids lie contiguously and padded to 4-entry slots. Per-tile start/length tables are replaced by piece offsets, per-tile deltas and per-256-record block flags. The probe kernel now walks flat 256-record blocks and scatters results through the tile delta. The collect kernel reads contiguous vectorized chunks instead of binary-searching tile bounds. This trades extra padding memory, new scan kernels and a changed sizing estimate for less indexing work and more coalesced loads; it also adds a debug export API.

After: 503.6 million. 4.4% lower.

```diff
diff --git a/commet_amd/csrc/capi/search_dispatch.hpp b/commet_amd/csrc/capi/search_dispatch.hpp
--- a/commet_amd/csrc/capi/search_dispatch.hpp
+++ b/commet_amd/csrc/capi/search_dispatch.hpp
@@ -315,6 +315,23 @@
 
 constexpr int TQ_MAX_K = 34;
 
+struct QueryListBounds { uint64_t entries, tiles, places, blocks; };
+inline QueryListBounds query_list_bounds(const commet_ctx *c, const commet_readset *rs)
+{
+    QueryListBounds b;
+    const uint64_t pieces = (rs->n_reads + TQ_PIECE - 1) / TQ_PIECE, records = rs->fhw_total;
+    b.entries = ((uint64_t) 1 << (c->k - TQ_SLICE_BITS)) * pieces;
+    b.tiles = std::min(b.entries, records);
+    b.places = records + 6 * b.tiles + 16 * pieces;
+    b.blocks = records / 256 + 2;
+    return b;
+}
+inline uint64_t query_list_tables(const commet_ctx *c, const commet_readset *rs)
+{
+    const QueryListBounds b = query_list_bounds(c, rs);
+    return (b.places - rs->fhw_total) * 2 + ((rs->n_reads + TQ_PIECE - 1) / TQ_PIECE + 1) * 8 + b.tiles * 4 + b.blocks * 4;
+}
+
 bool tiled_ok(const commet_ctx *c, const commet_readset *rs, int g)
 {
     if (c->tiled_mode == 1 || c->count_probes || rs->ql.failed) return false;
@@ -325,7 +342,7 @@
     if (rs->n_reads >= (1ull << 32)) return false;
     if (rs->fhw_total >= (1ull << 32)) return false;
     if (c->tiled_mode == 2) return true;
-    const uint64_t est = rs->fhw_total * 8;
+    const uint64_t est = rs->fhw_total * 8 + query_list_tables(c, rs);
     const bool set_aside = rs->ql_reserved.load() && rs->ql_reserved_at.load() == g_devmem.trims.load();
     if (rs->n_reads < (1ull << 20) || (est > c->ql_max_list && !set_aside)) return false;
     if (est > (4ull << 30) && !rs->ql.built && rs->ql_wanted++ == 0) return false;
@@ -340,12 +357,12 @@
         return 0;
     }
     ql.sbits = TQ_SLICE_BITS;
+    static_assert(TQ_SLICE_BITS <= 30, "qaddr keeps bits 30 and 31 for its flags");
     ql.n_slices = 1u << (c->k - ql.sbits);
     ql.n_pieces = (uint32_t) ((rs->n_reads + TQ_PIECE - 1) / TQ_PIECE);
     const uint64_t entries = (uint64_t) ql.n_slices * ql.n_pieces;
-    const uint32_t nb = (uint32_t) ((entries + 4095) / 4096);
+    const uint32_t nb = (uint32_t) ((entries + 4095) / 4096), nbp = (uint32_t) (((uint64_t) ql.n_pieces + 4095) / 4096);
     hipStream_t ls = c->list_stream;
-    unsigned long long *d_totals = nullptr;
     auto alloc = [&](void **ptr, size_t bytes) -> hipError_t {
         hipError_t ae = dm_malloc(ptr, bytes);
         if (ae != hipErrorOutOfMemory) return ae;
@@ -355,14 +372,17 @@
         if (ae == hipErrorOutOfMemory) (void) hipGetLastError();
         return ae;
     };
+    const uint64_t totals_need = (uint64_t) nb + 1 + nbp + 1;
     hipError_t e = alloc((void **) &ql.d_tile_off, (entries + 1) * sizeof(unsigned long long));
-    if (e == hipSuccess && c->ql_totals_cap < (uint64_t) nb + 1) {
+    if (e == hipSuccess) e = alloc((void **) &ql.d_piece_off, ((size_t) ql.n_pieces + 1) * sizeof(unsigned long long));
+    if (e == hipSuccess && c->ql_totals_cap < totals_need) {
         (void) dm_free(c->d_ql_totals);
         c->d_ql_totals = nullptr, c->ql_totals_cap = 0;
-        e = alloc((void **) &c->d_ql_totals, ((size_t) nb + 1) * sizeof(unsigned long long));
-        if (e == hipSuccess) c->ql_totals_cap = (uint64_t) nb + 1;
-    }
-    d_totals = c->d_ql_totals;
+        e = alloc((void **) &c->d_ql_totals, (size_t) totals_need * sizeof(unsigned long long));
+        if (e == hipSuccess) c->ql_totals_cap = totals_need;
+    }
+    unsigned long long *const d_totals = c->d_ql_totals, *const d_ptotals = d_totals + nb + 1;
+    uint64_t qaddr_cap = 0, blocks = 0;
     if (e == hipSuccess) {
         const int t = t_eff(c, rs);
         const size_t lds = (size_t) ql.n_slices * 4;
@@ -378,35 +398,41 @@
             COMMET_LAUNCH(tq_scan_blocks_kernel, dim3(nb), dim3(1024), 0, ls, ql.d_tile_off, entries, d_totals);
             COMMET_LAUNCH(tq_scan_totals_kernel, dim3(1), dim3(1024), 0, ls, d_totals, nb, d_totals + nb);
             COMMET_LAUNCH(tq_scan_add_kernel, dim3(nb), dim3(1024), 0, ls, ql.d_tile_off, entries, d_totals, d_totals + nb);
+            COMMET_LAUNCH(tq_piece_size_kernel, dim3(ql.n_pieces), dim3(256), 0, ls, ql.d_tile_off, ql.n_slices, ql.n_pieces, ql.d_piece_off);
+            COMMET_LAUNCH(tq_scan_blocks_kernel, dim3(nbp), dim3(1024), 0, ls, ql.d_piece_off, (uint64_t) ql.n_pieces, d_ptotals);
+            COMMET_LAUNCH(tq_scan_totals_kernel, dim3(1), dim3(1024), 0, ls, d_ptotals, nbp, d_ptotals + nbp);
+            COMMET_LAUNCH(tq_scan_add_kernel, dim3(nbp), dim3(1024), 0, ls, ql.d_piece_off, (uint64_t) ql.n_pieces, d_ptotals, d_ptotals + nbp);
         }
         e = hipGetLastError();
-        unsigned long long total = 0;
+        unsigned long long total = 0, places = 0;
         if (e == hipSuccess) e = hipMemcpyAsync(&total, d_totals + nb, sizeof total, hipMemcpyDeviceToHost, ls);
+        if (e == hipSuccess) e = hipMemcpyAsync(&places, d_ptotals + nbp, sizeof places, hipMemcpyDeviceToHost, ls);
         if (e == hipSuccess) e = hipStreamSynchronize(ls);
-        ql.n_records = total;
-        if (e == hipSuccess && total >= (1ull << 32)) e = hipErrorOutOfMemory;
-        if (e == hipSuccess) e = alloc((void **) &ql.d_qaddr, std::max<uint64_t>(total, 1) * 4);
-        if (e == hipSuccess) e = alloc((void **) &ql.d_qwho, std::max<uint64_t>(total, 1) * 2);
-        if (e == hipSuccess) e = alloc((void **) &ql.d_tstart, std::max<uint64_t>(entries, 1) * 4);
-        if (e == hipSuccess) e = alloc((void **) &ql.d_tlen, std::max<uint64_t>(entries, 1) * 2);
-        if (e == hipSuccess) {
-            KScope ks(c, "tq_bounds_kernel", ls);
-            COMMET_LAUNCH(tq_bounds_kernel, dim3((unsigned) ((entries + 255) / 256)), dim3(256), 0, ls, ql.d_tile_off, ql.n_slices,
-                               ql.n_pieces, ql.d_tstart, ql.d_tlen);
-            e = hipGetLastError();
-        }
+        ql.n_records = total & 0xFFFFFFFFull;
+        ql.n_tiles = total >> 32;
+        ql.n_places = places;
+        if (e == hipSuccess && places >= (1ull << 32)) e = hipErrorOutOfMemory;
+        blocks = ql.n_records / 256 + 2;
+        qaddr_cap = std::max<uint64_t>((ql.n_records + 255) / 256 * 256, 256);
+        if (e == hipSuccess) e = alloc((void **) &ql.d_qaddr, qaddr_cap * 4);
+        if (e == hipSuccess) e = alloc((void **) &ql.d_qwho, std::max<uint64_t>(ql.n_places, 16) * 2);
+        if (e == hipSuccess) e = alloc((void **) &ql.d_tile_delta, std::max<uint64_t>(ql.n_tiles, 1) * 4);
+        if (e == hipSuccess) e = alloc((void **) &ql.d_blk_first, blocks * 4);
+        if (e == hipSuccess) e = hipMemsetAsync(ql.d_qwho, 0xFF, std::max<uint64_t>(ql.n_places, 16) * 2, ls);
+        if (e == hipSuccess && qaddr_cap > ql.n_records) e = hipMemsetAsync(ql.d_qaddr + ql.n_records, 0, (qaddr_cap - ql.n_records) * 4, ls);
+        if (e == hipSuccess) e = hipMemsetAsync(ql.d_blk_first, 0, blocks * 4, ls);
         if (e == hipSuccess) {
             const int64_t fhw = std::max<int64_t>(1, (int64_t) rs->max_len - (int64_t) t * c->k + 1);
             const uint32_t rounds = (uint32_t) (((uint64_t) TQ_PIECE * (uint64_t) fhw + TQ_FILL_CAP - 1) / TQ_FILL_CAP);
             uint32_t rpr = (TQ_PIECE + rounds - 1) / rounds;
             while (rpr > 1 && (uint64_t) rpr * (uint64_t) fhw > TQ_FILL_CAP) --rpr;
-            const size_t lds_fill = ((size_t) 4 * ql.n_slices + 2 * TQ_FILL_CAP) * 4;
+            const size_t lds_fill = ((size_t) 5 * ql.n_slices + 2 * TQ_FILL_CAP) * 4;
             e = with_key(c->k, [&](auto key) {
                 hipError_t fe = hipFuncSetAttribute((const void *) tq_fill_kernel<decltype(key)>, hipFuncAttributeMaxDynamicSharedMemorySize, (int) lds_fill);
                 if (fe != hipSuccess) return fe;
                 KScope ks(c, "tq_fill_kernel", ls);
                 COMMET_LAUNCH(tq_fill_kernel<decltype(key)>, dim3(ql.n_pieces), dim3(256), lds_fill, ls, rs->view(), c->k, t, ql.sbits, ql.n_slices,
-                              ql.n_pieces, rpr, ql.d_tstart, ql.d_qaddr, ql.d_qwho);
+                              ql.n_pieces, rpr, ql.d_tile_off, ql.d_piece_off, ql.d_qaddr, ql.d_qwho, ql.d_tile_delta, ql.d_blk_first);
                 return hipGetLastError();
             });
         }
@@ -420,7 +446,8 @@
         return 1;
     }
     ql.built = true;
-    ql.bytes = (entries + 1) * 8 + ql.n_records * 6 + entries * 6;
+    ql.bytes = (entries + 1) * 8 + ((uint64_t) ql.n_pieces + 1) * 8 + qaddr_cap * 4 + std::max<uint64_t>(ql.n_places, 16) * 2 +
+               std::max<uint64_t>(ql.n_tiles, 1) * 4 + blocks * 4;
     ql.last_use = ++c->ql_clock;
     c->ql_bytes += ql.bytes;
     if (c->ql_bytes > c->ql_budget) (void) shrink_query_lists(c, c->ql_budget, false);
@@ -429,7 +456,7 @@
 
 int ensure_query_results(commet_ctx *c, const commet_readset *rs)
 {
-    const uint64_t need = rs->ql.n_records;
+    const uint64_t need = rs->ql.n_places;
     if (c->qres_cap >= need && c->d_qres) return 0;
     if (hipStreamSynchronize(c->stream) != hipSuccess) return 1;
     (void) dm_free(c->d_qres);
@@ -448,16 +475,18 @@
     return 0;
 }
 
-bool query_list_blocks(const commet_ctx *c, const commet_readset *rs, uint64_t out[6])
+constexpr int QL_BLOCKS = 7;
+bool query_list_blocks(const commet_ctx *c, const commet_readset *rs, uint64_t out[QL_BLOCKS])
 {
     const int t = t_eff(c, rs);
     const int64_t fhw = (int64_t) rs->max_len - (int64_t) t * c->k + 1;
     if (c->k <= TQ_SLICE_BITS || c->k > TQ_MAX_K || fhw < 1 || fhw > TQ_MAX_WIN || rs->max_len >= TQ_MAX_LEN || rs->n_reads < (1ull << 20) || rs->n_reads >= (1ull << 32)) return false;
     const uint64_t records = rs->fhw_total;
     if (records >= (1ull << 32)) return false;
-    const uint64_t entries = ((uint64_t) 1 << (c->k - TQ_SLICE_BITS)) * ((rs->n_reads + TQ_PIECE - 1) / TQ_PIECE);
-    out[0] = (entries + 1) * 8, out[1] = records * 4, out[2] = records * 2, out[3] = entries * 4, out[4] = entries * 2;
-    out[5] = c->qres_cap >= records ? 0 : records;
+    const QueryListBounds b = query_list_bounds(c, rs);
+    out[0] = (b.entries + 1) * 8, out[1] = (records + 255) / 256 * 256 * 4, out[2] = b.places * 2, out[3] = ((rs->n_reads + TQ_PIECE - 1) / TQ_PIECE + 1) * 8;
+    out[4] = b.tiles * 4, out[5] = b.blocks * 4;
+    out[6] = c->qres_cap >= b.places ? 0 : b.places;
     return true;
 }
 
@@ -468,9 +497,9 @@
 {
     if (rs->n_reads == 0) return 0;
     const commet_readset::QueryList &q = rs->ql;
-    if (c->qres_cap < q.n_records) return fail("internal error: tiled search without its result buffer");
+    if (c->qres_cap < q.n_places) return fail("internal error: tiled search without its result buffer");
     QueryListView v;
-    v.tile_off = q.d_tile_off, v.qaddr = q.d_qaddr, v.qwho = q.d_qwho, v.tstart = q.d_tstart, v.tlen = q.d_tlen;
+    v.tile_off = q.d_tile_off, v.qaddr = q.d_qaddr, v.qwho = q.d_qwho, v.piece_off = q.d_piece_off, v.tile_delta = q.d_tile_delta, v.blk_first = q.d_blk_first;
     v.n_slices = q.n_slices, v.n_pieces = q.n_pieces, v.sbits = q.sbits;
     FilterGroupView fg;
     fg.slot0 = c->slot_ptr(slot0);
@@ -483,7 +512,7 @@
     {
         KScope ks(c, "tq_probe_kernel", c->stream);
         with_value<1, 2>(g, [&](auto GS) {
-            COMMET_LAUNCH(tq_probe_kernel<GS>, dim3(8 * TQ_PROBE_WGS_PER_XCD), dim3(256), 0, c->stream, v, fg.il_a, c->d_qres, 0u, q.n_pieces);
+            COMMET_LAUNCH(tq_probe_kernel<GS>, dim3(8 * TQ_PROBE_WGS_PER_XCD), dim3(256), 0, c->stream, v, fg.il_a, c->d_qres);
         });
     }
     HIP_OK(hipGetLastError());
@@ -655,9 +684,9 @@
 
 uint64_t commet_readset_cache_estimate(commet_ctx *c, const commet_readset *rs)
 {
-    uint64_t b[6];
+    uint64_t b[QL_BLOCKS];
     if (rs->ctx != c || !rs->finalized || !query_list_blocks(c, rs, b)) return 0;
-    return b[0] + b[1] + b[2] + b[3] + b[4];
+    return b[0] + b[1] + b[2] + b[3] + b[4] + b[5];
 }
 
 int commet_readset_reserve_cache(commet_ctx *c, const commet_readset *rs)
@@ -667,17 +696,43 @@
     SetUse use(c, rs);
     if (use.enter()) return 1;
     HIP_OK(hipSetDevice(c->device));
-    uint64_t b[6];
+    uint64_t b[QL_BLOCKS];
     {
         std::lock_guard<std::mutex> lk(c->ql_mu);
         const bool still = rs->ql_reserved.load() && rs->ql_reserved_at.load() == g_devmem.trims.load();
         if (rs->ql.built || still || !g_devmem.enabled() || !query_list_blocks(c, rs, b)) return 0;
     }
-    for (int i = 0; i < 6; ++i)
+    for (int i = 0; i < QL_BLOCKS; ++i)
         if (b[i] && dm_reserve((size_t) b[i]) != hipSuccess) return 0;
     rs->ql_reserved_at.store(g_devmem.trims.load());
     rs->ql_reserved.store(true);
     return 0;
 }
 
-}
+int commet_readset_query_list(commet_ctx *c, const commet_readset *rs, uint64_t *dims, uint64_t *tile_off, uint32_t *qaddr, uint16_t *qwho,
+                              uint64_t *piece_off, uint32_t *tile_delta, uint32_t *blk_first)
+{
+    if (rs->ctx != c) return fail("read set belongs to another context");
+    if (!rs->finalized) return fail("read set not finalized");
+    SetUse use(c, rs);
+    if (use.enter()) return 1;
+    HIP_OK(hipSetDevice(c->device));
+    std::lock_guard<std::mutex> lk(c->ql_mu);
+    if (!tiled_ok(c, rs, 1) || build_query_list(c, rs) != 0) return fail("the set has no query list (tiled search not possible for it)");
+    HIP_OK(hipStreamSynchronize(c->list_stream));
+    const commet_readset::QueryList &q = rs->ql;
+    const uint64_t entries = (uint64_t) q.n_slices * q.n_pieces, blocks = q.n_records / 256 + 2, qaddr_n = std::max<uint64_t>((q.n_records + 255) / 256 * 256, 256);
+    if (dims) {
+        const uint64_t d[8] = {q.n_records, q.n_places, q.n_tiles, q.n_slices, q.n_pieces, (uint64_t) q.sbits, blocks, qaddr_n};
+        memcpy(dims, d, sizeof d);
+    }
+    if (tile_off) HIP_OK(hipMemcpy(tile_off, q.d_tile_off, (entries + 1) * 8, hipMemcpyDeviceToHost));
+    if (qaddr) HIP_OK(hipMemcpy(qaddr, q.d_qaddr, qaddr_n * 4, hipMemcpyDeviceToHost));
+    if (qwho && q.n_places) HIP_OK(hipMemcpy(qwho, q.d_qwho, q.n_places * 2, hipMemcpyDeviceToHost));
+    if (piece_off) HIP_OK(hipMemcpy(piece_off, q.d_piece_off, ((uint64_t) q.n_pieces + 1) * 8, hipMemcpyDeviceToHost));
+    if (tile_delta && q.n_tiles) HIP_OK(hipMemcpy(tile_delta, q.d_tile_delta, q.n_tiles * 4, hipMemcpyDeviceToHost));
+    if (blk_first) HIP_OK(hipMemcpy(blk_first, q.d_blk_first, blocks * 4, hipMemcpyDeviceToHost));
+    return 0;
+}
+
+}
diff --git a/commet_amd/csrc/capi/state.hpp b/commet_amd/csrc/capi/state.hpp
--- a/commet_amd/csrc/capi/state.hpp
+++ b/commet_amd/csrc/capi/state.hpp
@@ -560,17 +560,17 @@
     uint64_t uid = 0;
     uint64_t fhw_total = 0;
     struct QueryList {
-        unsigned long long *d_tile_off = nullptr;
-        uint32_t *d_qaddr = nullptr, *d_tstart = nullptr;
-        uint16_t *d_qwho = nullptr, *d_tlen = nullptr;
-        uint64_t n_records = 0;
+        unsigned long long *d_tile_off = nullptr, *d_piece_off = nullptr;
+        uint32_t *d_qaddr = nullptr, *d_tile_delta = nullptr, *d_blk_first = nullptr;
+        uint16_t *d_qwho = nullptr;
+        uint64_t n_records = 0, n_places = 0, n_tiles = 0;
         uint32_t n_slices = 0, n_pieces = 0;
         int sbits = 0;
         bool built = false, failed = false;
         uint64_t bytes = 0, last_use = 0;
         void release()
         {
-            (void) dm_free(d_tile_off); (void) dm_free(d_qaddr); (void) dm_free(d_qwho); (void) dm_free(d_tstart); (void) dm_free(d_tlen);
+            (void) dm_free(d_tile_off); (void) dm_free(d_piece_off); (void) dm_free(d_qaddr); (void) dm_free(d_qwho); (void) dm_free(d_tile_delta); (void) dm_free(d_blk_first);
             *this = QueryList();
         }
     };
diff --git a/commet_amd/csrc/tile_search.hpp b/commet_amd/csrc/tile_search.hpp
--- a/commet_amd/csrc/tile_search.hpp
+++ b/commet_amd/csrc/tile_search.hpp
@@ -6,21 +6,27 @@
 namespace commet {
 
 constexpr int TQ_SWEEP_U = 2;
-constexpr int TQ_COLLECT_U = 8;
+constexpr int TQ_COLLECT_U = 4;
 constexpr int TQ_HIT_CAP = 1024;
 constexpr uint32_t TQ_PIECE = 256;
 constexpr uint32_t TQ_MAX_LEN = 8000;
 constexpr int      TQ_MAX_WIN = 255;
+constexpr uint32_t TQ_PAD = 0xFFFFu;
+constexpr uint32_t TQ_FIRST = 0x40000000u, TQ_SELFP = 0x80000000u;
 
 struct QueryListView {
     const unsigned long long *tile_off;
     const uint32_t *qaddr;
     const uint16_t *qwho;
-    const uint32_t *tstart;
-    const uint16_t *tlen;
+    const unsigned long long *piece_off;
+    const uint32_t *tile_delta;
+    const uint32_t *blk_first;
     uint32_t n_slices, n_pieces;
     int sbits;
 };
+__device__ __forceinline__ uint32_t tq_lo(unsigned long long x) { return (uint32_t) x; }
+__device__ __forceinline__ uint32_t tq_hi(unsigned long long x) { return (uint32_t) (x >> 32); }
+__device__ __forceinline__ uint32_t tq_slot(uint32_t a, uint32_t len) { return len ? ((a & 3u) + len + 3u) & ~3u : 0u; }
 
 template <typename W, typename F>
 __device__ __forceinline__ void tq_for_each_window(const ReadsView &rv, uint64_t r, int k, int t, F &&f)
@@ -62,7 +68,21 @@
         tq_for_each_window<W>(rv, r, k, t, [&](uint32_t, W addr, bool) { atomicAdd(&h[(uint32_t) (addr >> sbits)], 1u); });
     }
     __syncthreads();
-    for (uint32_t s = threadIdx.x; s < n_slices; s += 256) cnt[(uint64_t) s * n_pieces + blockIdx.x] = h[s];
+    for (uint32_t s = threadIdx.x; s < n_slices; s += 256) cnt[(uint64_t) s * n_pieces + blockIdx.x] = h[s] | (h[s] ? 1ull << 32 : 0ull);
+}
+
+__global__ __launch_bounds__(256) void tq_piece_size_kernel(const unsigned long long *__restrict__ tile_off, uint32_t n_slices, uint32_t n_pieces,
+                                                            unsigned long long *__restrict__ psize)
+{
+    __shared__ uint32_t wsum[4];
+    uint32_t v = 0;
+    for (uint32_t s = threadIdx.x; s < n_slices; s += 256) {
+        const uint32_t a = tq_lo(tile_off[(uint64_t) s * n_pieces + blockIdx.x]), e = tq_lo(tile_off[(uint64_t) s * n_pieces + blockIdx.x + 1]);
+        v += tq_slot(a, e - a);
+    }
+    uint32_t tot;
+    (void) block_scan<256>(v, wsum, &tot);
+    if (threadIdx.x == 0) psize[blockIdx.x] = (tot + 15u) & ~15u;
 }
 
 __global__ __launch_bounds__(1024) void tq_scan_blocks_kernel(unsigned long long *__restrict__ a, uint64_t n, unsigned long long *__restrict__ totals)
@@ -180,30 +200,42 @@
     if (blockIdx.x == 0 && threadIdx.x == 0) ids[rv.n] = (uint32_t) rv.n;
 }
 
-__global__ __launch_bounds__(256) void tq_bounds_kernel(const unsigned long long *__restrict__ tile_off, uint32_t n_slices, uint32_t n_pieces,
-                                                        uint32_t *__restrict__ tstart, uint16_t *__restrict__ tlen)
-{
-    const uint64_t i = blockIdx.x * 256ull + threadIdx.x;
-    if (i >= (uint64_t) n_slices * n_pieces) return;
-    const uint64_t p = i / n_slices, s = i % n_slices;
-    const unsigned long long a = tile_off[s * n_pieces + p], e = tile_off[s * n_pieces + p + 1];
-    tstart[i] = (uint32_t) a;
-    tlen[i] = (uint16_t) (e - a);
-}
-
 constexpr uint32_t TQ_FILL_CAP = 9600;
 template <typename W>
 __global__ __launch_bounds__(256) void tq_fill_kernel(ReadsView rv, int k, int t, int sbits, uint32_t n_slices, uint32_t n_pieces,
-                                                      uint32_t rpr, const uint32_t *__restrict__ tstart,
-                                                      uint32_t *__restrict__ qaddr, uint16_t *__restrict__ qwho)
-{
-    static_assert(TQ_PIECE <= 256 && TQ_MAX_WIN <= 256, "qwho packs the read in 8 bits and the window in 8");
+                                                      uint32_t rpr, const unsigned long long *__restrict__ tile_off,
+                                                      const unsigned long long *__restrict__ piece_off,
+                                                      uint32_t *__restrict__ qaddr, uint16_t *__restrict__ qwho,
+                                                      uint32_t *__restrict__ tile_delta, uint32_t *__restrict__ blk_first)
+{
+    static_assert(TQ_PIECE <= 256 && TQ_MAX_WIN <= 255, "qwho packs the read in 8 bits and the window in 8; window 255 is TQ_PAD's");
     extern __shared__ uint32_t fl[];
-    uint32_t *cnt = fl, *base = cnt + n_slices, *fill = base + n_slices, *dstb = fill + n_slices;
-    uint32_t *rec_a = dstb + n_slices, *rec_w = rec_a + TQ_FILL_CAP;
+    uint32_t *cnt = fl, *base = cnt + n_slices, *fill = base + n_slices, *dstb = fill + n_slices, *dlt = dstb + n_slices;
+    uint32_t *rec_a = dlt + n_slices, *rec_w = rec_a + TQ_FILL_CAP;
     __shared__ uint32_t wsum[16];
     __shared__ uint32_t pw[TQ_PIECE + 1];
-    for (uint32_t i = threadIdx.x; i < n_slices; i += 256) dstb[i] = tstart[(uint64_t) blockIdx.x * n_slices + i];
+    for (uint32_t i = threadIdx.x; i < n_slices; i += 256) {
+        const uint32_t a = tq_lo(tile_off[(uint64_t) i * n_pieces + blockIdx.x]), e = tq_lo(tile_off[(uint64_t) i * n_pieces + blockIdx.x + 1]);
+        dstb[i] = a;
+        cnt[i] = tq_slot(a, e - a);
+    }
+    __syncthreads();
+    lds_scan<256>(cnt, base, n_slices, wsum);
+    {
+        const uint32_t pm0 = (uint32_t) piece_off[blockIdx.x];
+        for (uint32_t i = threadIdx.x; i < n_slices; i += 256) {
+            const unsigned long long x = tile_off[(uint64_t) i * n_pieces + blockIdx.x];
+            const uint32_t a = tq_lo(x), e = tq_lo(tile_off[(uint64_t) i * n_pieces + blockIdx.x + 1]);
+            const uint32_t d = pm0 + base[i] + (a & 3u) - a;
+            dlt[i] = d;
+            if (e == a) continue;
+            const uint32_t ord = tq_hi(x);
+            tile_delta[ord] = d;
+            for (uint32_t b = (a >> 8) + 1; b <= (e >> 8); ++b) blk_first[b] = ord + 1;
+        }
+        if (blockIdx.x == 0 && threadIdx.x == 0) blk_first[0] = 0;
+    }
+    __syncthreads();
     const uint64_t r0 = (uint64_t) blockIdx.x * TQ_PIECE;
     const uint32_t smask = (1u << sbits) - 1u;
     {
@@ -244,7 +276,7 @@
             tq_for_each_window<W>(rv, r0 + i, k, t, [&](uint32_t win, W addr, bool selfp) {
                 const uint32_t s = (uint32_t) (addr >> sbits);
                 const uint32_t at = base[s] + atomicAdd(&fill[s], 1u);
-                rec_a[at] = ((uint32_t) addr & smask) | (selfp ? 0x80000000u : 0u);
+                rec_a[at] = ((uint32_t) addr & smask) | (selfp ? TQ_SELFP : 0u);
                 rec_w[at] = i | (win << 8) | (s << 16);
             });
         __syncthreads();
@@ -252,8 +284,9 @@
         for (uint32_t j = threadIdx.x; j < total; j += 256) {
             const uint32_t w = rec_w[j], s = w >> 16;
             const uint32_t dst = dstb[s] + (j - base[s]);
-            qaddr[dst] = rec_a[j];
-            qwho[dst] = (uint16_t) (w & 0xFFFFu);
+            const bool first = j == base[s] && dst == tq_lo(tile_off[(uint64_t) s * n_pieces + blockIdx.x]);
+            qaddr[dst] = rec_a[j] | (first ? TQ_FIRST : 0u);
+            qwho[dst + dlt[s]] = (uint16_t) (w & 0xFFFFu);
         }
         __syncthreads();
         for (uint32_t s = threadIdx.x; s < n_slices; s += 256) dstb[s] += cnt[s];
@@ -263,7 +296,7 @@
 template <int GS>
 __device__ __forceinline__ uint32_t tq_probe_one(const uint32_t *__restrict__ base, uint32_t q)
 {
-    const uint32_t addr = q & 0x7FFFFFFFu, bit = addr & 31u;
+    const uint32_t addr = q & ~(TQ_SELFP | TQ_FIRST), bit = addr & 31u;
     const bool selfp = q >> 31;
     if constexpr (GS == 1) {
         const uint32_t wd = base[addr >> 5];
@@ -278,39 +311,43 @@
 }
 
 template <int GS>
-__global__ __launch_bounds__(256) void tq_probe_kernel(QueryListView ql, const uint32_t *__restrict__ planes_a, uint8_t *__restrict__ qres,
-                                                       uint32_t p0, uint32_t p1)
+__global__ __launch_bounds__(256) void tq_probe_kernel(QueryListView ql, const uint32_t *__restrict__ planes_a, uint8_t *__restrict__ qres)
 {
     const uint32_t x = blockIdx.x % 8, j = blockIdx.x / 8, wpx = gridDim.x / 8;
+    const uint32_t lane = threadIdx.x & 63, wave = j * 4 + (threadIdx.x >> 6), n_waves = wpx * 4;
     const uint32_t s_lo = (uint32_t) ((uint64_t) x * ql.n_slices / 8), s_hi = (uint32_t) ((uint64_t) (x + 1) * ql.n_slices / 8);
+    const unsigned long long lanes_before = (1ull << lane) - 1ull;
     for (uint32_t s = s_lo; s < s_hi; ++s) {
-        unsigned long long a = ql.tile_off[(uint64_t) s * ql.n_pieces + p0];
-        const unsigned long long e = ql.tile_off[(uint64_t) s * ql.n_pieces + p1];
+        const uint32_t a = tq_lo(ql.tile_off[(uint64_t) s * ql.n_pieces]), e = tq_lo(ql.tile_off[(uint64_t) (s + 1) * ql.n_pieces]);
+        if (a == e) continue;
         const uint32_t *base = planes_a + (((uint64_t) s << ql.sbits) >> 5) * GS;
-        const unsigned long long a4 = (a + 3) & ~3ull, e4 = e & ~3ull;
-        if (a4 < e4) {
-            const unsigned long long step = (unsigned long long) wpx * 256, m_end = e4 / 4;
-            unsigned long long m = a4 / 4 + (unsigned long long) j * 256 + threadIdx.x;
-            for (; m < m_end; m += step) {
-                const uint32_t *qp = ql.qaddr + 4 * m;
-                const uint32_t q0 = __builtin_nontemporal_load(qp), q1 = __builtin_nontemporal_load(qp + 1),
-                               q2 = __builtin_nontemporal_load(qp + 2), q3 = __builtin_nontemporal_load(qp + 3);
-                const uint32_t r = tq_probe_one<GS>(base, q0) | (tq_probe_one<GS>(base, q1) << 8) | (tq_probe_one<GS>(base, q2) << 16) |
-                                   (tq_probe_one<GS>(base, q3) << 24);
-                __builtin_nontemporal_store(r, (uint32_t *) (qres + 4 * m));
-            }
-        }
-        if (j == 0 && threadIdx.x < 8) {
-            unsigned long long i;
-            bool mine;
-            if (a4 < e4) {
-                i = threadIdx.x < 4 ? a + threadIdx.x : e4 + (threadIdx.x - 4);
-                mine = threadIdx.x < 4 ? i < a4 : i < e;
+        for (uint32_t blk = (a >> 8) + wave; blk <= ((e - 1u) >> 8); blk += n_waves) {
+            const uint32_t i0 = blk * 256u + 4u * lane;
+            const uint32_t *qp = ql.qaddr + i0;
+            uint32_t q[4];
+#pragma unroll
+            for (int u = 0; u < 4; ++u) q[u] = __builtin_nontemporal_load(qp + u);
+            uint32_t before = ql.blk_first[blk], fl[4];
+#pragma unroll
+            for (int u = 0; u < 4; ++u) {
+                fl[u] = (q[u] >> 30) & 1u;
+                before += (uint32_t) __popcll(__ballot(fl[u]) & lanes_before);
+            }
+            const uint32_t o0 = before + fl[0] - 1u;
+            if (i0 >= a && i0 + 3u < e && !(fl[1] | fl[2] | fl[3])) {
+                const uint32_t d = ql.tile_delta[o0];
+                const uint32_t r = tq_probe_one<GS>(base, q[0]) | (tq_probe_one<GS>(base, q[1]) << 8) | (tq_probe_one<GS>(base, q[2]) << 16) |
+                                   (tq_probe_one<GS>(base, q[3]) << 24);
+                __builtin_nontemporal_store(r, (uint32_t *) (qres + (uint32_t) (i0 + d)));
             } else {
-                i = a + threadIdx.x;
-                mine = i < e;
-            }
-            if (mine) qres[i] = (uint8_t) tq_probe_one<GS>(base, ql.qaddr[i]);
+                uint32_t o = o0 - fl[0];
+#pragma unroll
+                for (int u = 0; u < 4; ++u) {
+                    o += fl[u];
+                    const uint32_t i = i0 + (uint32_t) u;
+                    if (i >= a && i < e) qres[(uint32_t) (i + ql.tile_delta[o])] = (uint8_t) tq_probe_one<GS>(base, q[u]);
+                }
+            }
         }
     }
 }
@@ -328,58 +365,38 @@
     for (uint32_t i = threadIdx.x; i < GS * 2 * MW * TQ_PIECE; i += TQ_PIECE) masks[i] = 0;
     __syncthreads();
     {
-        const uint32_t lane = threadIdx.x & 63, wave = threadIdx.x >> 6;
-        constexpr uint32_t NWAVE = TQ_PIECE / 64;
-        for (uint32_t s0 = wave; s0 < ql.n_slices; s0 += 64 * NWAVE) {
-            const uint32_t sl = s0 + lane * NWAVE;
-            unsigned long long ta = 0, te = 0;
-            if (sl < ql.n_slices) {
-                ta = ql.tstart[(uint64_t) piece * ql.n_slices + sl];
-                te = ta + ql.tlen[(uint64_t) piece * ql.n_slices + sl];
-            }
-            const uint32_t len = (uint32_t) (te - ta);
-            uint32_t inc = len;
-            for (int o = 1; o < 64; o <<= 1) {
-                const uint32_t x = __shfl_up(inc, o, 64);
-                if ((int) lane >= o) inc += x;
-            }
-            const uint32_t total = __shfl(inc, 63, 64);
-            for (uint32_t f0 = 0; f0 < total; f0 += 64 * TQ_COLLECT_U) {
-                unsigned long long ri[TQ_COLLECT_U];
-                bool ok[TQ_COLLECT_U];
-#pragma unroll
-                for (int u = 0; u < TQ_COLLECT_U; ++u) {
-                    const uint32_t f = f0 + 64u * (uint32_t) u + lane;
-                    uint32_t lo = 0, hi = 64;
-#pragma unroll
-                    for (int step = 0; step < 7; ++step) {
-                        const uint32_t mid = min((lo + hi) >> 1, 63u);
-                        const uint32_t pm = __shfl(inc, (int) mid, 64);
-                        if (lo < hi) {
-                            if (pm <= f) lo = mid + 1;
-                            else hi = mid;
-                        }
-                    }
-                    const uint32_t src = min(lo, 63u);
-                    const uint32_t before_raw = __shfl(inc, (int) (src ? src - 1 : 0), 64);
-                    const unsigned long long tbase = __shfl((unsigned long long) ta, (int) src, 64);
-                    ok[u] = f < total;
-                    ri[u] = ok[u] ? tbase + (f - (src ? before_raw : 0u)) : 0ull;
+        typedef uint32_t u32x2 __attribute__((ext_vector_type(2)));
+        typedef uint32_t u32x4 __attribute__((ext_vector_type(4)));
+        const unsigned long long b0 = ql.piece_off[piece], b1 = ql.piece_off[piece + 1];
+        const uint32_t units = (uint32_t) ((b1 - b0) >> 3);
+        const u32x2 *const rp = (const u32x2 *) (qres + b0);
+        const u32x4 *const wp = (const u32x4 *) (ql.qwho + b0);
+        for (uint32_t u0 = threadIdx.x; u0 < units; u0 += TQ_COLLECT_U * TQ_PIECE) {
+            u32x2 res[TQ_COLLECT_U];
+            u32x4 who[TQ_COLLECT_U];
+#pragma unroll
+            for (int u = 0; u < TQ_COLLECT_U; ++u) {
+                const uint32_t at = u0 + (uint32_t) u * TQ_PIECE;
+                res[u] = u32x2{0u, 0u}, who[u] = u32x4{0u, 0u, 0u, 0u};
+                if (at < units) {
+                    res[u] = __builtin_nontemporal_load(rp + at);
+                    who[u] = __builtin_nontemporal_load(wp + at);
                 }
-                uint32_t res[TQ_COLLECT_U], who[TQ_COLLECT_U];
-#pragma unroll
-                for (int u = 0; u < TQ_COLLECT_U; ++u) {
-                    res[u] = __builtin_nontemporal_load(qres + ri[u]);
-                    who[u] = __builtin_nontemporal_load(ql.qwho + ri[u]);
-                }
-#pragma unroll
-                for (int u = 0; u < TQ_COLLECT_U; ++u) {
-                    if (!ok[u] || !res[u]) continue;
-                    const uint32_t rd = who[u] & 255u, win = who[u] >> 8;
+            }
+#pragma unroll
+            for (int u = 0; u < TQ_COLLECT_U; ++u) {
+                if (!(res[u].x | res[u].y)) continue;
+#pragma unroll
+                for (int b = 0; b < 8; ++b) {
+                    const uint32_t r = ((b < 4 ? res[u].x : res[u].y) >> (8 * (b & 3))) & 0xFFu;
+                    const uint32_t wq = b >> 1 == 0 ? who[u].x : b >> 1 == 1 ? who[u].y : b >> 1 == 2 ? who[u].z : who[u].w;
+                    const uint32_t w = (wq >> (16 * (b & 1))) & 0xFFFFu;
+                    if (!r || w == TQ_PAD) continue;
+                    const uint32_t rd = w & 255u, win = w >> 8;
 #pragma unroll
                     for (int c = 0; c < GS; ++c) {
-                        if ((res[u] >> c) & 1u) atomicOr(&mask_at(c, 0, (int) (win >> 5), rd), 1u << (win & 31u));
-                        if ((res[u] >> (GS + c)) & 1u) atomicOr(&mask_at(c, 1, (int) (win >> 5), rd), 1u << (win & 31u));
+                        if ((r >> c) & 1u) atomicOr(&mask_at(c, 0, (int) (win >> 5), rd), 1u << (win & 31u));
+                        if ((r >> (GS + c)) & 1u) atomicOr(&mask_at(c, 1, (int) (win >> 5), rd), 1u << (win & 31u));
                     }
                 }
             }
diff --git a/commet_amd/lib.py b/commet_amd/lib.py
--- a/commet_amd/lib.py
+++ b/commet_amd/lib.py
@@ -72,6 +72,7 @@
     "commet_cache_stats": (C.c_int, [C.c_void_p, u64p, u64p, u64p]),
     "commet_readset_cache_estimate": (C.c_uint64, [C.c_void_p, C.c_void_p]),
     "commet_readset_reserve_cache": (C.c_int, [C.c_void_p, C.c_void_p]),
+    "commet_readset_query_list": (C.c_int, [C.c_void_p, C.c_void_p, C.c_void_p, C.c_void_p, C.c_void_p, C.c_void_p, C.c_void_p, C.c_void_p, C.c_void_p]),
     "commet_device_cache_trim": (C.c_uint64, [C.c_int]),
     "commet_device_cache_bytes": (C.c_uint64, [C.c_int]),
     "commet_device_pooled_bytes": (C.c_uint64, [C.c_int]),
diff --git a/include/commet_hip.h b/include/commet_hip.h
--- a/include/commet_hip.h
+++ b/include/commet_hip.h
@@ -64,6 +64,8 @@
 uint64_t        commet_device_cache_trim(int device);
 uint64_t        commet_readset_cache_estimate(commet_ctx *ctx, const commet_readset *rs);
 int             commet_readset_reserve_cache(commet_ctx *ctx, const commet_readset *rs);
+int             commet_readset_query_list(commet_ctx *ctx, const commet_readset *rs, uint64_t *dims, uint64_t *tile_off, uint32_t *qaddr,
+                                          uint16_t *qwho, uint64_t *piece_off, uint32_t *tile_delta, uint32_t *blk_first);
 uint64_t        commet_device_cache_bytes(int device);
 uint64_t        commet_device_pooled_bytes(int device);
 int             commet_device_alloc_stats(int device, double *wait_ms, uint64_t *fresh_bytes, uint64_t *calls);
```
